# LuizGuzzo/Monocular_Depth_Estimation

Hardware: AMD Instinct MI355X
Metric: training images/sec at 640x480 bs=32/GPU (GuideDepth, SSIM+0.1*L1, Adam) (higher is better)
Workload: dtype fp32; 1 GPU; GuideDepth (DDRNet-23-slim + 3 guided upsampling blocks) train step, BASELINE cfg2, BN in train mode; global_batch=32, per_gpu_batch=32, resolution=640x480, parallelism=dp1

## Files before the change

include/mde_abi.h:

```cpp
#ifndef MDE_ABI_H
#define MDE_ABI_H

#include <stddef.h>
#include <stdint.h>

#ifdef __cplusplus
extern "C" {
#endif

#define MDE_ABI_VERSION 1

#define MDE_F32 0
#define MDE_BF16 1

#define MDE_OK 0
#define MDE_ERR_INVALID_ARG (-1)
#define MDE_ERR_UNSUPPORTED (-2)

int mde_abi_version(void);
const char* mde_status_string(int status);


int mde_bilinear_fwd(const void* x, void* y, int64_t n, int64_t c, int64_t hi,
                     int64_t wi, int64_t ho, int64_t wo, float scale_h,
// ... 64 lines not shown
                        int64_t w, void* workspace, int dtype, void* stream);
int mde_skip_reduce_bn_supported(int64_t cin, int64_t cout, int64_t h, int64_t w, int sums);
size_t mde_skip_reduce_bn_workspace(int64_t n, int64_t cin, int64_t cout, int64_t h, int64_t w);
int mde_skip_reduce_bn_fwd(const void* r, const void* d, const float* in_scale,
                           const float* in_shift, const float* wt, const float* b, void* out,
                           int64_t n, int64_t cin, int64_t cout, int64_t h, int64_t w, int dtype,
                           void* stream);
int mde_skip_reduce_bn_bwd(const void* gout, const void* r, const void* d, const float* in_scale,
                           const float* in_shift, const float* in_mean, const float* wt, void* gs,
                           float* gw, float* gb, float* in_sums, int64_t n, int64_t cin,
                           int64_t cout, int64_t h, int64_t w, void* workspace, int dtype,
                           void* stream);

size_t mde_minmax_workspace(int64_t numel);
int mde_minmax(const void* x, int64_t numel, float* minmax, void* workspace,
               int dtype, void* stream);
int mde_depthnorm_apply(const void* x, const float* minmax, void* y,
                        int64_t numel, int dtype, void* stream);

size_t mde_ssim3_l1_workspace(int64_t b, int64_t h, int64_t w);
int mde_ssim3_l1_fwd(const void* pred, const void* target,
                     const float* target_minmax, float w_ssim, float w_l1,
                     float* loss, void* grad_pred, void* grad_target,
                     int64_t b, int64_t h, int64_t w, void* workspace,
                     int dtype, void* stream);

size_t mde_depth_loss_workspace(int64_t b, int64_t h, int64_t w);
int mde_depth_loss_fwd(const void* pred, const void* gt, float alpha,
                       float beta, float gamma, float max_depth, float* out,
                       int64_t b, int64_t h, int64_t w, void* workspace,
                       int dtype, void* stream);
int mde_depth_loss_bwd(const void* pred, const void* gt, float alpha,
                       float beta, float gamma, float max_depth,
                       const float* fwd_out, const float* gout,
                       void* grad_pred, int64_t b, int64_t h, int64_t w,
                       void* workspace, int dtype, void* stream);

size_t mde_batchnorm_workspace(int64_t n, int64_t c, int64_t h, int64_t w);
int mde_batchnorm_fwd_train(const void* x, const float* gamma, const float* beta,
                            const float* prebias, float* running_mean,
                            float* running_var, int64_t* num_batches_tracked,
                            float momentum, float eps, const void* residual,
                            void* y, float* save_mean, float* save_invstd,
                            int64_t n, int64_t c, int64_t h, int64_t w, int act,
                            void* workspace, int dtype, void* stream);
int mde_batchnorm_fwd_eval(const void* x, const float* gamma, const float* beta,
                           const float* prebias, const float* running_mean,
                           const float* running_var, float eps,
                           const void* residual, void* y, float* save_mean,
                           float* save_invstd, int64_t n, int64_t c, int64_t h,
                           int64_t w, int act, int dtype, void* stream);
int mde_batchnorm_fwd_coef(const void* x, const float* gamma, const float* beta,
                           const float* prebias, float* running_mean, float* running_var,
                           int64_t* num_batches_tracked, float momentum, float eps,
                           int training, float* scale, float* shift, float* save_mean,
                           float* save_invstd, int64_t n, int64_t c, int64_t h, int64_t w,
                           void* workspace, int dtype, void* stream);
int mde_batchnorm_bwd(const void* gy, const void* x, const void* residual,
                      const float* gamma, const float* beta, const float* mean,
                      const float* invstd, int training, void* gx,
                      void* gresidual, float* ggamma, float* gbeta,
                      float* gprebias, int64_t n, int64_t c, int64_t h,
                      int64_t w, int act, void* workspace, int dtype,
                      void* stream);
int mde_batchnorm_fwd_train_stats(const void* x, const float* gamma, const float* beta,
                                  const float* prebias, float* running_mean, float* running_var,
                                  int64_t* num_batches_tracked, float momentum, float eps,
                                  const void* residual, void* y, float* save_mean,
                                  float* save_invstd, int64_t n, int64_t c, int64_t h, int64_t w,
                                  int act, const float* stats, int64_t stats_blocks,
                                  void* workspace, int dtype, void* stream);
int mde_batchnorm_fwd_coef_stats(const void* x, const float* gamma, const float* beta,
                                 const float* prebias, float* running_mean, float* running_var,
                                 int64_t* num_batches_tracked, float momentum, float eps,
                                 float* scale, float* shift, float* save_mean, float* save_invstd,
                                 int64_t n, int64_t c, int64_t h, int64_t w, const float* stats,
                                 int64_t stats_blocks, void* workspace, int dtype, void* stream);
int mde_batchnorm_bwd_apply(const void* gy, const void* x, const void* residual,
                            const float* gamma, const float* beta, const float* mean,
                            const float* invstd, int training, const float* sums, void* gx,
                            void* gresidual, float* ggamma, float* gbeta, float* gprebias,
                            int64_t n, int64_t c, int64_t h, int64_t w, int act, int dtype,
                            void* stream);

size_t mde_window_attn_workspace(int64_t b, int64_t h, int64_t w, int64_t c,
                                 int64_t heads, int64_t window);
int mde_window_attn_fwd(const void* qk, const float* qk_bias, const void* v,
                        const float* v_bias, const float* table, void* out, int64_t b,
                        int64_t h, int64_t w, int64_t c, int64_t heads, int64_t window,
                        int64_t shift, int dtype, void* stream);
int mde_window_attn_bwd(const void* gout, const void* qk, const float* qk_bias,
                        const void* v, const float* v_bias, const float* table, void* gqk,
                        void* gv, float* gtable, float* gqk_bias, float* gv_bias, int64_t b,
                        int64_t h, int64_t w, int64_t c, int64_t heads, int64_t window,
                        int64_t shift, void* workspace, int dtype, void* stream);

size_t mde_colsum_workspace(int64_t t_rows, int64_t n);
int mde_colsum(const void* g, float* gb, int64_t t_rows, int64_t n, void* workspace, int dtype,
               void* stream);
int mde_gelu_bwd_colsum(const void* dh, const void* a, void* da, float* gb, int64_t t_rows,
                        int64_t n, void* workspace, int dtype, void* stream);

size_t mde_linear_wgrad_workspace(int64_t t_rows, int64_t m, int64_t n);
int mde_linear_wgrad(const void* g, const void* x, float* gw, float* gb, int64_t t_rows,
                     int64_t m, int64_t n, void* workspace, int dtype, void* stream);

size_t mde_chansum_workspace(int64_t n, int64_t c, int64_t hw);
int mde_chansum(const void* g, float* gb, int64_t n, int64_t c, int64_t hw, void* workspace,
                int dtype, void* stream);

int mde_head_conv_supported(int64_t n, int64_t c, int64_t h, int64_t w);
int mde_head_conv_fwd(const void* x, const float* weight, const float* bias, void* y, int64_t n,
                      int64_t c, int64_t h, int64_t w, int dtype, void* stream);
int mde_head_conv_dgrad(const void* gy, const float* weight, void* gx, int64_t n, int64_t c,
                        int64_t h, int64_t w, int dtype, void* stream);
size_t mde_head_conv_wgrad_workspace(int64_t n, int64_t c, int64_t h, int64_t w);
int mde_head_conv_wgrad(const void* gy, const void* x, float* gweight, int64_t n, int64_t c,
                        int64_t h, int64_t w, void* workspace, int dtype, void* stream);

int mde_pointwise_supported(int64_t cin, int64_t cout, int64_t h, int64_t w);
size_t mde_pointwise_workspace(int64_t n, int64_t cin, int64_t cout, int64_t h, int64_t w);
int mde_pointwise_fwd(const void* x, const float* in_scale, const float* in_shift,
                      const float* weight, void* y, int64_t n, int64_t cin, int64_t cout,
                      int64_t h, int64_t w, int dtype, void* stream);
int mde_pointwise_bwd(const void* gy, const void* x, const float* in_scale,
                      const float* in_shift, const float* weight, void* gx, float* gweight,
                      int64_t n, int64_t cin, int64_t cout, int64_t h, int64_t w,
                      void* workspace, int dtype, void* stream);
int mde_pointwise_stats_blocks(int64_t n, int64_t cin, int64_t cout, int64_t h, int64_t w);
int mde_pointwise_fwd_stats(const void* x, const float* in_scale, const float* in_shift,
                            const float* weight, void* y, float* stats, int64_t n, int64_t cin,
                            int64_t cout, int64_t h, int64_t w, int dtype, void* stream);
int mde_pointwise_bwd_bn(const void* gy, const void* x, const float* in_scale,
                         const float* in_shift, const float* in_mean, const float* weight,
                         void* gx, float* gweight, float* in_sums, int64_t n, int64_t cin,
                         int64_t cout, int64_t h, int64_t w, void* workspace, int dtype,
                         void* stream);

int mde_conv3x3_supported(int64_t cin, int64_t cout, int pass, int dtype);
int mde_conv3x3_fwd(const void* x, const float* weight, void* y, int64_t n, int64_t cin,
                    int64_t cout, int64_t h, int64_t w, int dtype, void* stream);
int mde_conv3x3_stats_blocks(int64_t n, int64_t cin, int64_t cout, int64_t h, int64_t w,
                             int dtype);
int mde_conv3x3_fwd_stats(const void* x, const float* weight, void* y, float* stats, int64_t n,
                          int64_t cin, int64_t cout, int64_t h, int64_t w, int dtype,
                          void* stream);
int mde_conv3x3_bwd_data(const void* gy, const float* weight, void* gx, int64_t n,
                         int64_t cin, int64_t cout, int64_t h, int64_t w, int dtype,
                         void* stream);
size_t mde_conv3x3_wgrad_workspace(int64_t n, int64_t cin, int64_t cout, int64_t h, int64_t w,
                                   int dtype);
int mde_conv3x3_wgrad(const void* gy, const void* x, float* gweight, int64_t n, int64_t cin,
                      int64_t cout, int64_t h, int64_t w, void* workspace, int dtype,
                      void* stream);

int mde_conv3x3s2_supported(int64_t cin, int64_t cout, int dtype);
size_t mde_conv3x3s2_wgrad_workspace(int64_t n, int64_t cin, int64_t cout, int64_t h, int64_t w,
                                     int dtype);
int mde_conv3x3s2_wgrad(const void* gy, const void* x, float* gweight, int64_t n, int64_t cin,
                        int64_t cout, int64_t h, int64_t w, void* workspace, int dtype,
                        void* stream);

size_t mde_dwconv_workspace(int64_t n, int64_t c, int64_t h, int64_t w, int64_t k,
                            int64_t stride, int64_t pad);
int mde_dwconv_fwd(const void* x, const float* weight, void* y, int64_t n, int64_t c,
                   int64_t h, int64_t w, int64_t k, int64_t stride, int64_t pad, int dtype,
                   void* stream);
int mde_dwconv_bwd(const void* gy, const void* x, const float* weight, void* gx,
                   float* gweight, int64_t n, int64_t c, int64_t h, int64_t w, int64_t k,
                   int64_t stride, int64_t pad, void* workspace, int dtype, void* stream);

size_t mde_layernorm_workspace(int64_t rows, int64_t c);
int mde_layernorm_fwd(const void* x, const float* gamma, const float* beta, void* y,
                      float* mean, float* rstd, int64_t rows, int64_t c, float eps, int dtype,
                      void* stream);
int mde_layernorm_bwd(const void* gy, const void* x, const float* gamma, const float* mean,
                      const float* rstd, void* gx, float* ggamma, float* gbeta, int64_t rows,
                      int64_t c, void* workspace, int dtype, void* stream);
int mde_layernorm_add_fwd(const void* x, const void* r, const float* gamma, const float* beta,
                          void* sum, void* y, float* mean, float* rstd, int64_t rows, int64_t c,
                          float eps, int dtype, void* stream);
int mde_layernorm_bwd_res(const void* gy, const void* x, const void* gres, const float* gamma,
                          const float* mean, const float* rstd, void* gx, float* ggamma,
                          float* gbeta, int64_t rows, int64_t c, void* workspace, int dtype,
                          void* stream);

int mde_transpose(const void* x, void* y, int64_t batch, int64_t m, int64_t n, int dtype,
                  void* stream);

int mde_nyu_augment(const void* image, const void* depth, const int32_t* flags, float* image_out,
                    float* depth_out, int64_t n, int64_t h, int64_t w, int64_t dh, int64_t dw,
                    int depth_bits, void* stream);

size_t mde_eval_workspace(int64_t n, int64_t h, int64_t w);
int mde_eval_sums(const void* pred, const void* gt, int64_t n, int64_t h, int64_t w,
                  float min_depth, float max_depth, int mode, const int32_t* crop,
                  void* workspace, double* sums, int dtype, void* stream);

int mde_conv3x3_guide_bf16_stats_blocks(int64_t n, int64_t cout, int64_t h, int64_t w);
int mde_conv3x3_guide_bf16_fwd(const float* x, const float* weight, void* y, float* stats,
                               int64_t n, int64_t cout, int64_t h, int64_t w, void* stream);

int mde_conv1x1_supported(int64_t cin, int64_t cout, int64_t h, int64_t w, int stride,
                          int dtype);
int mde_conv1x1_fwd(const void* x, const float* weight, void* y, int64_t n, int64_t cin,
                    int64_t cout, int64_t h, int64_t w, int stride, int dtype, void* stream);
int mde_conv1x1_bwd_data(const void* gy, const float* weight, void* gx, int64_t n, int64_t cin,
                         int64_t cout, int64_t h, int64_t w, int stride, int dtype,
                         void* stream);
size_t mde_conv1x1_wgrad_workspace(int64_t n, int64_t cin, int64_t cout, int64_t h, int64_t w,
                                   int stride, int dtype);
int mde_conv1x1_wgrad(const void* gy, const void* x, float* gweight, int64_t n, int64_t cin,
                      int64_t cout, int64_t h, int64_t w, int stride, void* workspace, int dtype,
                      void* stream);

int mde_conv3x3s2_fwd_supported(int64_t cin, int64_t cout, int64_t h, int64_t w, int dtype);
int mde_conv3x3s2_dgrad_supported(int64_t cin, int64_t cout, int64_t h, int64_t w, int dtype);
int mde_conv3x3s2_fwd(const void* x, const float* weight, void* y, int64_t n, int64_t cin,
                      int64_t cout, int64_t h, int64_t w, int dtype, void* stream);
int mde_conv3x3s2_bwd_data(const void* gy, const float* weight, void* gx, int64_t n, int64_t cin,
                           int64_t cout, int64_t h, int64_t w, int dtype, void* stream);

int mde_conv3x3_wide_supported(int64_t cin, int64_t cout, int64_t h, int64_t w, int pass,
                               int dtype);
int mde_conv3x3_wide_fwd(const void* x, const float* weight, void* y, int64_t n, int64_t cin,
                         int64_t cout, int64_t h, int64_t w, int dtype, void* stream);
int mde_conv3x3_wide_bwd_data(const void* gy, const float* weight, void* gx, int64_t n,
                              int64_t cin, int64_t cout, int64_t h, int64_t w, int dtype,
                              void* stream);

int mde_wino_mode(int mode);
int mde_wino_supported(int64_t cin, int64_t cout, int64_t h, int64_t w, int dtype);
size_t mde_wino_weight_bytes(int64_t cin, int64_t cout);
int mde_wino_weight(const float* weight, float* u, int64_t cin, int64_t cout, int flip,
                    void* stream);
int mde_wino_weight2(const float* weight, float* u, float* u_flip, int64_t cin, int64_t cout,
                     void* stream);
// ... 76 lines not shown
```

monocular_depth_estimation_amd/_abi.py:

```python
from __future__ import annotations

import ctypes
import os

import torch

LIB_PATH = os.environ.get("MDE_HIP_LIB") or os.path.join(
    os.path.dirname(os.path.abspath(__file__)), "libmde_hip.so")

MDE_F32 = 0
MDE_BF16 = 1

_c = ctypes
_vp = _c.c_void_p
_i64 = _c.c_int64
_f32 = _c.c_float
_int = _c.c_int
_sz = _c.c_size_t
_fp = _c.POINTER(_c.c_float)

SIGNATURES = {
    "mde_abi_version": (_int, []),
    "mde_status_string": (_c.c_char_p, [_int]),
    "mde_bilinear_fwd": (_int, [_vp, _vp, _i64, _i64, _i64, _i64, _i64, _i64, _f32, _f32, _int, _int, _vp]),
    "mde_bilinear_bwd": (_int, [_vp, _vp, _i64, _i64, _i64, _i64, _i64, _i64, _f32, _f32, _int, _int, _vp]),
    "mde_bilinear_bwd2_supported": (_int, [_i64, _i64, _i64, _i64, _i64, _i64, _f32, _f32, _int]),
    "mde_bilinear_bwd2": (_int, [_vp, _vp, _vp, _i64, _i64, _i64, _i64, _i64, _i64, _f32, _f32, _int,
                                 _int, _vp]),
    "mde_nearest_fwd": (_int, [_vp, _vp, _i64, _i64, _i64, _i64, _i64, _i64, _f32, _f32, _int, _vp]),
    "mde_nearest_bwd": (_int, [_vp, _vp, _i64, _i64, _i64, _i64, _i64, _i64, _f32, _f32, _int, _vp]),
    "mde_nearest_pyramid_supported": (_int, [_i64, _i64, _i64, _i64]),
    "mde_nearest_pyramid": (_int, [_vp, _vp, _vp, _i64, _i64, _i64, _i64, _int, _vp]),
    "mde_se_workspace": (_sz, [_i64, _i64, _i64, _i64, _i64]),
    "mde_se_fwd": (_int, [_vp, _i64, _vp, _i64, _vp, _vp, _i64, _vp, _vp, _vp, _vp,
                          _i64, _i64, _i64, _vp, _int, _vp]),
    "mde_se_bwd": (_int, [_vp, _vp, _i64, _vp, _i64, _vp, _vp, _i64, _vp, _vp, _vp,
                          _vp, _vp, _vp, _vp, _i64, _i64, _i64, _vp, _int, _vp]),
    "mde_se_bn_workspace": (_sz, [_i64, _i64, _i64, _i64, _i64]),
    "mde_se_bn_fwd": (_int, [_vp, _i64, _vp, _i64, _vp, _vp, _vp, _vp, _i64, _vp, _vp, _vp, _vp,
                             _i64, _i64, _i64, _vp, _int, _vp]),
    "mde_se_bn_bwd": (_int, [_vp, _vp, _i64, _vp, _i64, _vp, _vp, _vp, _vp, _int, _vp, _vp, _i64,
                             _vp, _vp, _vp, _vp, _vp, _vp, _vp, _vp, _vp, _i64, _i64, _i64, _vp,
                             _int, _vp]),
    "mde_skip_reduce_fwd": (_int, [_vp, _vp, _vp, _vp, _vp, _i64, _i64, _i64, _i64, _i64, _int, _vp]),
    "mde_skip_reduce_workspace": (_sz, [_i64, _i64, _i64, _i64, _i64]),
    "mde_skip_reduce_bwd": (_int, [_vp, _vp, _vp, _vp, _vp, _vp, _vp, _i64, _i64, _i64, _i64, _i64,
                                   _vp, _int, _vp]),
    "mde_skip_reduce_bn_supported": (_int, [_i64, _i64, _i64, _i64, _int]),
    "mde_skip_reduce_bn_workspace": (_sz, [_i64, _i64, _i64, _i64, _i64]),
    "mde_skip_reduce_bn_fwd": (_int, [_vp, _vp, _vp, _vp, _vp, _vp, _vp, _i64, _i64, _i64, _i64, _i64,
                                      _int, _vp]),
    "mde_skip_reduce_bn_bwd": (_int, [_vp, _vp, _vp, _vp, _vp, _vp, _vp, _vp, _vp, _vp, _vp, _i64,
                                      _i64, _i64, _i64, _i64, _vp, _int, _vp]),
    "mde_minmax_workspace": (_sz, [_i64]),
    "mde_minmax": (_int, [_vp, _i64, _vp, _vp, _int, _vp]),
    "mde_depthnorm_apply": (_int, [_vp, _vp, _vp, _i64, _int, _vp]),
    "mde_ssim3_l1_workspace": (_sz, [_i64, _i64, _i64]),
    "mde_ssim3_l1_fwd": (_int, [_vp, _vp, _vp, _f32, _f32, _vp, _vp, _vp, _i64, _i64, _i64, _vp, _int, _vp]),
    "mde_depth_loss_workspace": (_sz, [_i64, _i64, _i64]),
    "mde_depth_loss_fwd": (_int, [_vp, _vp, _f32, _f32, _f32, _f32, _vp, _i64, _i64, _i64, _vp, _int, _vp]),
    "mde_depth_loss_bwd": (_int, [_vp, _vp, _f32, _f32, _f32, _f32, _vp, _vp, _vp, _i64, _i64, _i64,
                                  _vp, _int, _vp]),
    "mde_batchnorm_workspace": (_sz, [_i64, _i64, _i64, _i64]),
    "mde_batchnorm_fwd_train": (_int, [_vp, _vp, _vp, _vp, _vp, _vp, _vp, _f32, _f32, _vp, _vp, _vp,
                                       _vp, _i64, _i64, _i64, _i64, _int, _vp, _int, _vp]),
    "mde_batchnorm_fwd_eval": (_int, [_vp, _vp, _vp, _vp, _vp, _vp, _f32, _vp, _vp, _vp, _vp,
                                      _i64, _i64, _i64, _i64, _int, _int, _vp]),
    "mde_batchnorm_bwd": (_int, [_vp, _vp, _vp, _vp, _vp, _vp, _vp, _int, _vp, _vp, _vp, _vp, _vp,
                                 _i64, _i64, _i64, _i64, _int, _vp, _int, _vp]),
    "mde_batchnorm_bwd_apply": (_int, [_vp, _vp, _vp, _vp, _vp, _vp, _vp, _int, _vp, _vp, _vp, _vp,
                                       _vp, _vp, _i64, _i64, _i64, _i64, _int, _int, _vp]),
    "mde_window_attn_workspace": (_sz, [_i64, _i64, _i64, _i64, _i64, _i64]),
    "mde_window_attn_fwd": (_int, [_vp, _vp, _vp, _vp, _vp, _vp, _i64, _i64, _i64, _i64, _i64, _i64,
                                   _i64, _int, _vp]),
    "mde_window_attn_bwd": (_int, [_vp, _vp, _vp, _vp, _vp, _vp, _vp, _vp, _vp, _vp, _vp, _i64, _i64,
                                   _i64, _i64, _i64, _i64, _i64, _vp, _int, _vp]),
    "mde_se_gate_fwd": (_int, [_vp, _i64, _vp, _i64, _vp, _vp, _vp, _vp, _i64, _int, _vp, _vp, _vp,
                               _vp, _i64, _i64, _i64, _vp, _int, _vp]),
    "mde_se_gate_bwd": (_int, [_vp, _vp, _i64, _vp, _i64, _vp, _vp, _vp, _i64, _int, _vp, _vp, _vp,
                               _vp, _vp, _vp, _vp, _vp, _vp, _i64, _i64, _i64, _vp, _int, _vp]),
    "mde_pointwise_supported": (_int, [_i64, _i64, _i64, _i64]),
    "mde_pointwise_workspace": (_sz, [_i64, _i64, _i64, _i64, _i64]),
    "mde_pointwise_fwd": (_int, [_vp, _vp, _vp, _vp, _vp, _i64, _i64, _i64, _i64, _i64, _int, _vp]),
    "mde_pointwise_bwd": (_int, [_vp, _vp, _vp, _vp, _vp, _vp, _vp, _i64, _i64, _i64, _i64, _i64,
                                 _vp, _int, _vp]),
    "mde_pointwise_stats_blocks": (_int, [_i64, _i64, _i64, _i64, _i64]),
    "mde_pointwise_fwd_stats": (_int, [_vp, _vp, _vp, _vp, _vp, _vp, _i64, _i64, _i64, _i64, _i64,
                                       _int, _vp]),
    "mde_conv3x3_stats_blocks": (_int, [_i64, _i64, _i64, _i64, _i64, _int]),
    "mde_conv3x3_fwd_stats": (_int, [_vp, _vp, _vp, _vp, _i64, _i64, _i64, _i64, _i64, _int, _vp]),
    "mde_batchnorm_fwd_train_stats": (_int, [_vp, _vp, _vp, _vp, _vp, _vp, _vp, _f32, _f32, _vp,
                                             _vp, _vp, _vp, _i64, _i64, _i64, _i64, _int, _vp,
                                             _i64, _vp, _int, _vp]),
    "mde_batchnorm_fwd_coef_stats": (_int, [_vp, _vp, _vp, _vp, _vp, _vp, _vp, _f32, _f32, _vp,
                                            _vp, _vp, _vp, _i64, _i64, _i64, _i64, _vp, _i64, _vp,
                                            _int, _vp]),
    "mde_pointwise_bwd_bn": (_int, [_vp, _vp, _vp, _vp, _vp, _vp, _vp, _vp, _vp, _i64, _i64, _i64,
                                    _i64, _i64, _vp, _int, _vp]),
    "mde_batchnorm_fwd_coef": (_int, [_vp, _vp, _vp, _vp, _vp, _vp, _vp, _f32, _f32, _int, _vp, _vp,
                                      _vp, _vp, _i64, _i64, _i64, _i64, _vp, _int, _vp]),
    "mde_conv3x3_supported": (_int, [_i64, _i64, _int, _int]),
    "mde_conv3x3_fwd": (_int, [_vp, _vp, _vp, _i64, _i64, _i64, _i64, _i64, _int, _vp]),
    "mde_conv3x3_bwd_data": (_int, [_vp, _vp, _vp, _i64, _i64, _i64, _i64, _i64, _int, _vp]),
    "mde_conv3x3_wgrad_workspace": (_sz, [_i64, _i64, _i64, _i64, _i64, _int]),
    "mde_conv3x3_wgrad": (_int, [_vp, _vp, _vp, _i64, _i64, _i64, _i64, _i64, _vp, _int, _vp]),
    "mde_conv3x3s2_supported": (_int, [_i64, _i64, _int]),
    "mde_conv3x3s2_wgrad_workspace": (_sz, [_i64, _i64, _i64, _i64, _i64, _int]),
    "mde_conv3x3s2_wgrad": (_int, [_vp, _vp, _vp, _i64, _i64, _i64, _i64, _i64, _vp, _int, _vp]),
    "mde_dwconv_workspace": (_sz, [_i64, _i64, _i64, _i64, _i64, _i64, _i64]),
    "mde_dwconv_fwd": (_int, [_vp, _vp, _vp, _i64, _i64, _i64, _i64, _i64, _i64, _i64, _int, _vp]),
    "mde_dwconv_bwd": (_int, [_vp, _vp, _vp, _vp, _vp, _i64, _i64, _i64, _i64, _i64, _i64, _i64,
                              _vp, _int, _vp]),
    "mde_layernorm_workspace": (_sz, [_i64, _i64]),
    "mde_layernorm_fwd": (_int, [_vp, _vp, _vp, _vp, _vp, _vp, _i64, _i64, _f32, _int, _vp]),
    "mde_layernorm_bwd": (_int, [_vp, _vp, _vp, _vp, _vp, _vp, _vp, _vp, _i64, _i64, _vp, _int,
                                 _vp]),
    "mde_layernorm_add_fwd": (_int, [_vp, _vp, _vp, _vp, _vp, _vp, _vp, _vp, _i64, _i64, _f32,
                                      _int, _vp]),
    "mde_layernorm_bwd_res": (_int, [_vp, _vp, _vp, _vp, _vp, _vp, _vp, _vp, _vp, _i64, _i64,
                                      _vp, _int, _vp]),
    "mde_transpose": (_int, [_vp, _vp, _i64, _i64, _i64, _int, _vp]),
    "mde_nyu_augment": (_int, [_vp, _vp, _vp, _vp, _vp, _i64, _i64, _i64, _i64, _i64, _int, _vp]),
    "mde_eval_workspace": (_sz, [_i64, _i64, _i64]),
    "mde_eval_sums": (_int, [_vp, _vp, _i64, _i64, _i64, _f32, _f32, _int, _c.POINTER(_c.c_int32), _vp,
                             _vp, _int, _vp]),
    "mde_colsum_workspace": (_sz, [_i64, _i64]),
    "mde_colsum": (_int, [_vp, _vp, _i64, _i64, _vp, _int, _vp]),
    "mde_head_conv_supported": (_int, [_i64, _i64, _i64, _i64]),
    "mde_head_conv_fwd": (_int, [_vp, _vp, _vp, _vp, _i64, _i64, _i64, _i64, _int, _vp]),
    "mde_head_conv_dgrad": (_int, [_vp, _vp, _vp, _i64, _i64, _i64, _i64, _int, _vp]),
    "mde_head_conv_wgrad_workspace": (_sz, [_i64, _i64, _i64, _i64]),
    "mde_head_conv_wgrad": (_int, [_vp, _vp, _vp, _i64, _i64, _i64, _i64, _vp, _int, _vp]),
    "mde_chansum_workspace": (_sz, [_i64, _i64, _i64]),
    "mde_chansum": (_int, [_vp, _vp, _i64, _i64, _i64, _vp, _int, _vp]),
    "mde_linear_wgrad_workspace": (_sz, [_i64, _i64, _i64]),
    "mde_linear_wgrad": (_int, [_vp, _vp, _vp, _vp, _i64, _i64, _i64, _vp, _int, _vp]),
    "mde_gelu_bwd_colsum": (_int, [_vp, _vp, _vp, _vp, _i64, _i64, _vp, _int, _vp]),
    "mde_conv1x1_supported": (_int, [_i64, _i64, _i64, _i64, _int, _int]),
    "mde_conv1x1_fwd": (_int, [_vp, _vp, _vp, _i64, _i64, _i64, _i64, _i64, _int, _int, _vp]),
    "mde_conv1x1_bwd_data": (_int, [_vp, _vp, _vp, _i64, _i64, _i64, _i64, _i64, _int, _int, _vp]),
    "mde_conv1x1_wgrad_workspace": (_sz, [_i64, _i64, _i64, _i64, _i64, _int, _int]),
    "mde_conv1x1_wgrad": (_int, [_vp, _vp, _vp, _i64, _i64, _i64, _i64, _i64, _int, _vp, _int,
                                 _vp]),
    "mde_conv3x3s2_fwd_supported": (_int, [_i64, _i64, _i64, _i64, _int]),
    "mde_conv3x3s2_dgrad_supported": (_int, [_i64, _i64, _i64, _i64, _int]),
    "mde_conv3x3s2_fwd": (_int, [_vp, _vp, _vp, _i64, _i64, _i64, _i64, _i64, _int, _vp]),
    "mde_conv3x3s2_bwd_data": (_int, [_vp, _vp, _vp, _i64, _i64, _i64, _i64, _i64, _int, _vp]),
    "mde_conv3x3_wide_supported": (_int, [_i64, _i64, _i64, _i64, _int, _int]),
    "mde_conv3x3_wide_fwd": (_int, [_vp, _vp, _vp, _i64, _i64, _i64, _i64, _i64, _int, _vp]),
    "mde_conv3x3_wide_bwd_data": (_int, [_vp, _vp, _vp, _i64, _i64, _i64, _i64, _i64, _int, _vp]),
    "mde_wino_mode": (_int, [_int]),
    "mde_wino_supported": (_int, [_i64, _i64, _i64, _i64, _int]),
    "mde_wino_weight_bytes": (_sz, [_i64, _i64]),
    "mde_wino_weight": (_int, [_vp, _vp, _i64, _i64, _int, _vp]),
    "mde_wino_weight2": (_int, [_vp, _vp, _vp, _i64, _i64, _vp]),
    "mde_wino_weight_blocks": (_i64, [_i64, _i64, _int]),
    "mde_wino_weight_table": (_int, [_vp, _int, _i64, _i64, _vp]),
    "mde_wino_conv": (_int, [_vp, _vp, _vp, _i64, _i64, _i64, _i64, _i64, _int, _int, _vp]),
    "mde_wino_conv_acc": (_int, [_vp, _vp, _vp, _vp, _i64, _i64, _i64, _i64, _i64, _int, _int, _vp]),
    "mde_wino_conv_stats": (_int, [_vp, _vp, _vp, _vp, _i64, _i64, _i64, _i64, _i64, _int, _int,
                                   _vp]),
    "mde_wino_stats_blocks": (_int, [_i64, _i64, _i64, _i64, _i64]),
    "mde_batchnorm_stats_route": (_int, [_i64, _i64, _i64, _i64, _i64, _int]),
    "mde_bn_chan_mode": (_int, [_int]),
    "mde_convbf_supported": (_int, [_i64, _i64, _i64, _i64, _int, _int, _int]),
    "mde_convbf_supported_n": (_int, [_i64, _i64, _i64, _i64, _i64, _int, _int, _int]),
    "mde_convbf_flops": (_c.c_double, [_i64, _i64, _i64, _i64, _i64, _int, _int, _int]),
    "mde_stem_bf16_supported": (_int, [_i64, _i64, _i64, _i64]),
    "mde_stem_bf16_fwd": (_int, [_vp, _vp, _vp, _i64, _i64, _i64, _i64, _vp]),
    "mde_stem_bf16_wgrad_workspace": (_sz, [_i64, _i64, _i64, _i64]),
    "mde_stem_bf16_wgrad": (_int, [_vp, _vp, _vp, _i64, _i64, _i64, _i64, _vp, _vp]),
    "mde_conv3x3_guide_bf16_wgrad_workspace": (_sz, [_i64, _i64, _i64, _i64]),
    "mde_conv3x3_guide_bf16_wgrad": (_int, [_vp, _vp, _vp, _i64, _i64, _i64, _i64, _vp, _vp]),
    "mde_convbf_pack_elems": (_sz, [_i64, _i64, _int, _int]),
    "mde_convbf_pack": (_int, [_vp, _vp, _i64, _i64, _int, _int, _vp]),
    "mde_convbf_pack_both": (_int, [_vp, _vp, _vp, _i64, _i64, _int, _vp]),
    "mde_convbf_pack_table": (_int, [_vp, _int, _i64, _i64, _vp]),
    "mde_convbf_stats_blocks": (_int, [_i64, _i64, _i64, _i64, _i64, _int, _int]),
    "mde_convbf_fwd": (_int, [_vp, _vp, _vp, _vp, _i64, _i64, _i64, _i64, _i64, _int, _int, _vp]),
    "mde_convbf_bwd_data": (_int, [_vp, _vp, _vp, _i64, _i64, _i64, _i64, _i64, _int, _int, _vp]),
    "mde_convbf_wgrad_workspace": (_sz, [_i64, _i64, _i64, _i64, _i64, _int, _int]),
    "mde_convbf_wgrad": (_int, [_vp, _vp, _vp, _i64, _i64, _i64, _i64, _i64, _int, _int, _vp, _vp]),
    "mde_conv3x3_guide_bf16_stats_blocks": (_int, [_i64, _i64, _i64, _i64]),
    "mde_conv3x3_guide_bf16_fwd": (_int, [_vp, _vp, _vp, _vp, _i64, _i64, _i64, _i64, _vp]),
    "mde_graph_count_memsets": (_int, [_vp, _c.POINTER(_i64)]),
    "mde_graph_replace_memsets": (_int, [_vp, _c.POINTER(_i64)]),
    "mde_graph_node_counts": (_int, [_vp, _c.POINTER(_i64)]),
    "mde_graph_node_types": (_int, [_vp, _c.POINTER(_i64)]),
# ... 153 lines not shown
```

monocular_depth_estimation_amd/csrc/bn.hip:

```cpp
#include <cmath>

#include <cstdlib>
#include <type_traits>

#include "common.h"

namespace {

constexpr int kTarget = 2048;
constexpr int kMinSlice = 4096;
constexpr int kPlaneChunk4 = 1024;
constexpr int64_t kMaxApplyRecords = 256;

struct Geo {
  int64_t c, hw, total;
  int slices;
  int64_t slice_len;
};

int64_t env_or(const char* name, int64_t dflt) {
  const char* v = std::getenv(name);
  return v && *v ? std::atoll(v) : dflt;
}

// ... 411 lines not shown
};

struct BwdCh {
  float sc, sh, A, B, D;
};

__device__ BwdCh bwd_channel(const BwdArgs& P, int64_t ch, double sdy,
                             double sdyx, bool owner) {
  BwdCh r;
  const double is = (double)P.invstd[ch];
  const double mu = (double)P.mean[ch];
  const double scale = (double)P.gamma[ch] * is;
  double A = scale, B = 0.0, D = 0.0;
  const double n = (double)P.total;
  if (P.training) {
    B = -scale * is * is * sdyx / n;
    D = -scale * sdy / n - B * mu;
  }
  if (owner) {
    if (P.ggamma) P.ggamma[ch] = (float)(sdyx * is);
    if (P.gbeta) P.gbeta[ch] = (float)sdy;
    if (P.gprebias) P.gprebias[ch] = (float)(A * sdy + B * n * mu + D * n);
  }
  r.sc = P.gamma[ch] * P.invstd[ch];
  r.sh = P.beta[ch] - P.mean[ch] * r.sc;
  r.A = (float)A;
  r.B = (float)B;
  r.D = (float)D;
  return r;
}

template <typename T>
__global__ void __launch_bounds__(256)
    bn_bwd_apply_plane_kernel(const T* __restrict__ gy, const T* __restrict__ x,
                              const T* __restrict__ r, T* __restrict__ gx,
                              T* __restrict__ gr, int64_t c, int64_t hw, int act,
                              BwdArgs P) {
  __shared__ float cf[5];
  const int64_t plane = blockIdx.y;
  const int64_t ch = plane % c;
  const int64_t hw4 = hw >> 2;
  const T* gp = gy + plane * hw;
  const T* xp = x + plane * hw;
  const T* rp = r ? r + plane * hw : nullptr;
  T* op = gx + plane * hw;
  T* orp = gr ? gr + plane * hw : nullptr;
  const int64_t b0 = blockIdx.x * (int64_t)kPlaneChunk4;
  constexpr int KK = kPlaneChunk4 / 256;
  float4 g4[KK], v4[KK], q4[KK];
#pragma unroll
  for (int k = 0; k < KK; ++k) {
    const int64_t i = b0 + k * 256 + threadIdx.x;
    const int64_t ic = i < hw4 ? i : hw4 - 1;
    g4[k] = ld4_nt(gp + 4 * ic);
    v4[k] = ld4_nt(xp + 4 * ic);
    q4[k] = rp ? ld4_nt(rp + 4 * ic) : make_float4(0.f, 0.f, 0.f, 0.f);
  }
  if (threadIdx.x < 64) {
    double a, b;
    wave_slices(P.part, ch, P.slices, &a, &b);
    if (threadIdx.x == 0) {
      const BwdCh k = bwd_channel(P, ch, a, b, blockIdx.x == 0 && plane < c);
      cf[0] = k.sc; cf[1] = k.sh; cf[2] = k.A; cf[3] = k.B; cf[4] = k.D;
    }
  }
  __syncthreads();
  const float sc = cf[0], sh = cf[1], A = cf[2], B = cf[3], D = cf[4];
#pragma unroll
  for (int k = 0; k < KK; ++k) {
    const int64_t i = b0 + k * 256 + threadIdx.x;
    if (i < hw4) {
      const float4 g = g4[k], v = v4[k], q = q4[k];
      const float4 e = make_float4(dy_eff(g.x, v.x, q.x, sc, sh, act),
                                   dy_eff(g.y, v.y, q.y, sc, sh, act),
                                   dy_eff(g.z, v.z, q.z, sc, sh, act),
                                   dy_eff(g.w, v.w, q.w, sc, sh, act));
      st4_nt(op + 4 * i, make_float4(A * e.x + B * v.x + D, A * e.y + B * v.y + D,
                                     A * e.z + B * v.z + D, A * e.w + B * v.w + D));
      if (orp) st4_nt(orp + 4 * i, e);
    }
  }
}

template <typename T>
__global__ void __launch_bounds__(256)
    bn_bwd_apply_table_kernel(const T* __restrict__ gy, const T* __restrict__ x,
                              const T* __restrict__ r, T* __restrict__ gx,
                              T* __restrict__ gr, int64_t planes, int64_t c,
                              int64_t hw, int act, BwdArgs P) {
  extern __shared__ float tab[];
  const PlaneShare ps(planes, c);
  for (int64_t kk = threadIdx.x; kk < ps.nch; kk += blockDim.x) {
    const int64_t ch = ps.channel(kk, c);
    double a = 0.0, b = 0.0;
    for (int s = 0; s < P.slices; ++s) {
      a += (double)P.part[(ch * P.slices + s) * 2];
      b += (double)P.part[(ch * P.slices + s) * 2 + 1];
    }
    const BwdCh k = bwd_channel(P, ch, a, b, ps.owner(ch));
    tab[ch] = k.sc;
    tab[c + ch] = k.sh;
    tab[2 * c + ch] = k.A;
    tab[3 * c + ch] = k.B;
    tab[4 * c + ch] = k.D;
  }
  __syncthreads();
  const int64_t total = planes * hw;
  if (table_vec(total, hw)) {
    const uint32_t hw4 = (uint32_t)(hw >> 2), cc = (uint32_t)c;
    const uint32_t t1 = (uint32_t)(ps.p1 * (hw >> 2));
    for (uint32_t t = (uint32_t)(ps.p0 * (hw >> 2)) + threadIdx.x; t < t1; t += blockDim.x) {
      const uint32_t ch = (t / hw4) % cc;
      const int64_t o = 4 * (int64_t)t;
      const float sc = tab[ch], sh = tab[c + ch];
      const float A = tab[2 * c + ch], B = tab[3 * c + ch], D = tab[4 * c + ch];
      const float4 v = ld4(x + o), g = ld4(gy + o);
      const float4 q = r ? ld4(r + o) : make_float4(0.f, 0.f, 0.f, 0.f);
      float4 e, o4;
      e.x = dy_eff(g.x, v.x, q.x, sc, sh, act);
      e.y = dy_eff(g.y, v.y, q.y, sc, sh, act);
      e.z = dy_eff(g.z, v.z, q.z, sc, sh, act);
      e.w = dy_eff(g.w, v.w, q.w, sc, sh, act);
      o4.x = A * e.x + B * v.x + D;
      o4.y = A * e.y + B * v.y + D;
      o4.z = A * e.z + B * v.z + D;
      o4.w = A * e.w + B * v.w + D;
      st4(gx + o, o4);
      if (gr) st4(gr + o, e);
    }
    return;
  }
  for (int64_t t = ps.p0 * hw + threadIdx.x; t < ps.p1 * hw; t += blockDim.x) {
    const int64_t ch = (t / hw) % c;
    const float v = ld1(x + t);
    const float e = dy_eff(ld1(gy + t), v, r ? ld1(r + t) : 0.f, tab[ch], tab[c + ch], act);
    st1(gx + t, tab[2 * c + ch] * e + tab[3 * c + ch] * v + tab[4 * c + ch]);
    if (gr) st1(gr + t, e);
  }
}

constexpr int kChanThreads = 512;
constexpr int kChanUnits = 8;
constexpr int64_t kChanMax = (int64_t)kChanThreads * kChanUnits * 4;

int g_chan_mode = [] {
  const char* e = std::getenv("MDE_BN_CHAN");
  return e ? std::atoi(e) : 2;
}();

template <typename T>
inline bool chan_mode(int64_t n, int64_t hw) {
  const bool on = std::is_same_v<T, float> ? g_chan_mode >= 1 : g_chan_mode >= 2;
  return on && !plane_mode(hw) && n * hw <= (hw % 4 == 0 ? kChanMax : kChanMax / 4);
}

__device__ __forceinline__ void chan_sum2(double* a, double* b, double (*red)[kChanThreads / 64]) {
  const int lane = threadIdx.x & 63, wv = threadIdx.x >> 6;
  double x = wave_sum_d(*a), y = wave_sum_d(*b);
  if (lane == 0) {
    red[0][wv] = x;
    red[1][wv] = y;
  }
  __syncthreads();
  x = 0.0;
  y = 0.0;
#pragma unroll
// ... 460 lines not shown
  if (!dtype_ok(dtype)) return MDE_ERR_UNSUPPORTED;
  if (!x || !gamma || !beta || !y || !save_mean || !save_invstd || !workspace || !stats ||
      stats_blocks <= 0 || stats_blocks > 0x7fffffff || (!running_mean != !running_var) ||
      act < 0 || act > 2 || !args_ok(n, c, h, w))
    return MDE_ERR_INVALID_ARG;
  hipStream_t s = (hipStream_t)stream;
  const int64_t hw = h * w;
  if (dtype == MDE_BF16 ? chan_mode<bf16>(n, hw) : chan_mode<float>(n, hw))
    return mde_batchnorm_fwd_train(x, gamma, beta, prebias, running_mean, running_var,
                                   num_batches_tracked, momentum, eps, residual, y, save_mean,
                                   save_invstd, n, c, h, w, act, workspace, dtype, stream);
  float* part = (float*)workspace;
  if (plane_mode(hw) && stats_blocks <= kMaxApplyRecords) {
    FwdArgs A{gamma, beta, prebias, part, 0, n * hw, hw, eps, momentum, running_mean,
              running_var, num_batches_tracked, save_mean, save_invstd, 1, stats,
              (int)stats_blocks};
    if (dtype == MDE_BF16)
      return launch_fwd_apply((const bf16*)x, (const bf16*)residual, (bf16*)y, n, c, hw, act, A, s);
    return launch_fwd_apply((const float*)x, (const float*)residual, (float*)y, n, c, hw, act, A, s);
  }
  const double mb = 16.0 * (double)c * stats_blocks;
  if (dtype == MDE_BF16)
    MDE_LAUNCH(mde::K_BN_FINAL, mb, s, (bn_stats_merge_kernel<bf16, false>), dim3((unsigned)c),
               dim3(256), 0, (const bf16*)x, stats, (int)stats_blocks, hw, part, FwdArgs{},
               nullptr, nullptr);
  else
    MDE_LAUNCH(mde::K_BN_FINAL, mb, s, (bn_stats_merge_kernel<float, false>), dim3((unsigned)c),
               dim3(256), 0, (const float*)x, stats, (int)stats_blocks, hw, part, FwdArgs{},
               nullptr, nullptr);
  FwdArgs A{gamma, beta, prebias, part, 1, n * hw, hw, eps, momentum,
            running_mean, running_var, num_batches_tracked, save_mean, save_invstd, 1};
  if (dtype == MDE_BF16)
    return launch_fwd_apply((const bf16*)x, (const bf16*)residual, (bf16*)y, n, c, hw, act, A, s);
  return launch_fwd_apply((const float*)x, (const float*)residual, (float*)y, n, c, hw, act, A, s);
}

int mde_batchnorm_fwd_coef_stats(const void* x, const float* gamma, const float* beta,
                                 const float* prebias, float* running_mean, float* running_var,
                                 int64_t* num_batches_tracked, float momentum, float eps,
                                 float* scale, float* shift, float* save_mean, float* save_invstd,
                                 int64_t n, int64_t c, int64_t h, int64_t w, const float* stats,
                                 int64_t stats_blocks, void* workspace, int dtype, void* stream) {
  if (!dtype_ok(dtype)) return MDE_ERR_UNSUPPORTED;
  if (!x || !gamma || !beta || !scale || !shift || !save_mean || !save_invstd || !workspace ||
      !stats || stats_blocks <= 0 || stats_blocks > 0x7fffffff ||
      (!running_mean != !running_var) || !args_ok(n, c, h, w))
    return MDE_ERR_INVALID_ARG;
  hipStream_t s = (hipStream_t)stream;
  const int64_t hw = h * w;
  float* part = (float*)workspace;
  const double mb = 16.0 * (double)c * stats_blocks;
  FwdArgs A{gamma, beta, prebias, part, 1, n * hw, hw, eps, momentum, running_mean, running_var,
            num_batches_tracked, save_mean, save_invstd, 1};
  if (dtype == MDE_BF16) {
    MDE_LAUNCH(mde::K_BN_FINAL, mb + 8.0 * (double)c, s, (bn_stats_merge_kernel<bf16, true>),
               dim3((unsigned)c), dim3(256), 0, (const bf16*)x, stats, (int)stats_blocks, hw,
               part, A, scale, shift);
  } else {
    MDE_LAUNCH(mde::K_BN_FINAL, mb + 8.0 * (double)c, s, (bn_stats_merge_kernel<float, true>),
               dim3((unsigned)c), dim3(256), 0, (const float*)x, stats, (int)stats_blocks, hw,
               part, A, scale, shift);
  }
  return MDE_OK;
}

int mde_batchnorm_bwd_apply(const void* gy, const void* x, const void* residual,
                            const float* gamma, const float* beta, const float* mean,
                            const float* invstd, int training, const float* sums, void* gx,
                            void* gresidual, float* ggamma, float* gbeta, float* gprebias,
                            int64_t n, int64_t c, int64_t h, int64_t w, int act, int dtype,
                            void* stream) {
  if (!dtype_ok(dtype)) return MDE_ERR_UNSUPPORTED;
  if (!gy || !x || !gamma || !beta || !mean || !invstd || !sums || !gx || act < 0 || act > 2 ||
      !args_ok(n, c, h, w) || (gresidual && !residual && act))
    return MDE_ERR_INVALID_ARG;
  hipStream_t s = (hipStream_t)stream;
  const int64_t hw = h * w;
  BwdArgs P{gamma, beta, mean, invstd, sums, 1, n * hw, training, ggamma, gbeta, gprebias};
  return dtype == MDE_BF16
             ? bwd_apply<bf16>(gy, x, residual, gx, gresidual, n, c, hw, act, P, s)
             : bwd_apply<float>(gy, x, residual, gx, gresidual, n, c, hw, act, P, s);
}

}
```

monocular_depth_estimation_amd/csrc/conv3x3.hip:

```cpp
#include <cstdlib>

#include "common.h"

namespace {

using f4 = __attribute__((__vector_size__(4 * sizeof(float)))) float;

__device__ __forceinline__ f4 mfma4(float a, float b, f4 c) {
  return __builtin_amdgcn_mfma_f32_16x16x4f32(a, b, c, 0, 0, 0);
}

__device__ __forceinline__ int clampi(int v, int lo, int hi) { return v < lo ? lo : (v > hi ? hi : v); }

template <auto Kernel>
int resident_blocks() {
  static const int cached = [] {
    int dev = 0, cus = 0, per = 0;
    (void)hipGetDevice(&dev);
    (void)hipDeviceGetAttribute(&cus, hipDeviceAttributeMultiprocessorCount, dev);
    (void)hipOccupancyMaxActiveBlocksPerMultiprocessor(&per, Kernel, 256, 0);
    return (cus > 0 ? cus : 256) * (per > 0 ? per : 1);
  }();
  return cached;
}

constexpr int kTW = 64;
constexpr int kXW = kTW + 2;

constexpr int cpad4(int c) { return (c + 3) / 4 * 4; }
constexpr int plane_words(int rows, int mod) { return (rows * kXW + 63) / 64 * 64 + mod; }
constexpr int wrow_words(int co) { return co == 16 ? 16 : (co == 32 ? 48 : 80); }

__device__ __forceinline__ float rbf(float v) {
  return __uint_as_float((uint32_t)__builtin_bit_cast(uint16_t, (__bf16)v) << 16);
}

template <int CI, int CIP, int XR>
struct HaloTile {
  static constexpr int ROWS = CIP * XR;
  static constexpr int RPWV = (ROWS + 3) / 4;
  static constexpr int NH = (2 * RPWV + 63) / 64;
  static_assert(RPWV <= 64 && NH <= 32, "mask widths");
  float a[RPWV];
  float b[NH];
  uint64_t am;
  unsigned bm;

  __device__ __forceinline__ void load(const float* __restrict__ xi, int h, int w, int r0,
                                       int c0, int lane, int wvu) {
    const int gc = c0 - 1 + lane;
    const bool cok = gc >= 0 && gc < w;
    am = 0;
#pragma unroll
    for (int k = 0; k < RPWV; ++k) {
      const int ri = wvu + 4 * k;
      const int c = ri / XR, r = ri % XR, gr = r0 - 1 + r;
      const bool ok = (ROWS % 4 == 0 || ri < ROWS) && (CI == CIP || c < CI) && gr >= 0 &&
                      gr < h && cok;
      a[k] = xi[ok ? (unsigned)((c * h + gr) * w + gc) : 0u];
      am |= ok ? (uint64_t)1 << k : (uint64_t)0;
    }
    bm = 0;
#pragma unroll
    for (int q = 0; q < NH; ++q) {
      const int e = 64 * q + lane;
      const int ri = wvu + 4 * (e >> 1);
      const int c = ri / XR, r = ri % XR, gr = r0 - 1 + r, g2 = c0 + 63 + (e & 1);
      const bool ok = e < 2 * RPWV && ri < ROWS && c < CI && gr >= 0 && gr < h && g2 < w;
      b[q] = xi[ok ? (unsigned)((c * h + gr) * w + g2) : 0u];
      bm |= ok ? 1u << q : 0u;
    }
  }

  template <int PS, bool RB = false>
  __device__ __forceinline__ void store(float* sx, int lane, int wvu) const {
#pragma unroll
    for (int k = 0; k < RPWV; ++k) {
      const int ri = wvu + 4 * k;
      if (ROWS % 4 == 0 || ri < ROWS) {
        const float v = (am >> k) & 1 ? a[k] : 0.f;
        sx[(ri / XR) * PS + (ri % XR) * kXW + lane] = RB ? rbf(v) : v;
      }
    }
#pragma unroll
    for (int q = 0; q < NH; ++q) {
      const int e = 64 * q + lane;
      const int ri = wvu + 4 * (e >> 1);
      if (e < 2 * RPWV && ri < ROWS) {
        const float v = (bm >> q) & 1u ? b[q] : 0.f;
        sx[(ri / XR) * PS + (ri % XR) * kXW + 64 + (e & 1)] = RB ? rbf(v) : v;
      }
    }
  }
};

template <int CO, int TH, bool FULL>
struct GradTile {
  static constexpr int ROWS = CO * TH;
  static constexpr int PER = (ROWS + 15) / 16;
  static_assert(PER <= 32, "mask width");
  float4 v[PER];
  unsigned vm;

  __device__ __forceinline__ void load(const float* __restrict__ gi, int h, int w, int r0,
                                       int c0, int lane, int wvu) {
    const int gc = c0 + 4 * (lane & 15);
    vm = 0;
#pragma unroll
    for (int i = 0; i < PER; ++i) {
      const int ri = 16 * i + 4 * wvu + (lane >> 4);
      const int c = ri / TH, gr = r0 + ri % TH;
      const bool rok = (ROWS % 16 == 0 || ri < ROWS) && gr < h;
      if constexpr (FULL) {
        v[i] = *reinterpret_cast<const float4*>(gi + (rok ? (unsigned)((c * h + gr) * w + gc) : 0u));
        vm |= rok ? 1u << i : 0u;
      } else {
        const float* src = gi + (rok ? ((int64_t)c * h + gr) * w + gc : 0);
        const bool vec = (w & 3) == 0 && gc + 3 < w;
        if (vec) {
          const float4 t = *reinterpret_cast<const float4*>(src);
          v[i] = rok ? t : make_float4(0.f, 0.f, 0.f, 0.f);
        } else {
          float4 t;
          t.x = rok && gc < w ? src[0] : 0.f;
          t.y = rok && gc + 1 < w ? src[1] : 0.f;
          t.z = rok && gc + 2 < w ? src[2] : 0.f;
          t.w = rok && gc + 3 < w ? src[3] : 0.f;
          v[i] = t;
        }
      }
    }
  }

  template <int PSG>
  __device__ __forceinline__ void store(float* sg, int lane, int wvu) const {
#pragma unroll
    for (int i = 0; i < PER; ++i) {
      const int ri = 16 * i + 4 * wvu + (lane >> 4);
      if (ROWS % 16 == 0 || ri < ROWS) {
        float4 t = v[i];
        if (FULL && !((vm >> i) & 1u)) t = make_float4(0.f, 0.f, 0.f, 0.f);
        *reinterpret_cast<float4*>(sg + (ri / TH) * PSG + (ri % TH) * kTW + 4 * (lane & 15)) = t;
      }
    }
  }
};

struct TileGeo {
  int img, r0, c0;
};

struct TileWalk {
  int t0, step, end;
};

__device__ __forceinline__ TileWalk tile_walk(int ntiles) {
  const int b = blockIdx.x, g = gridDim.x;
  if (g % 8 != 0 || ntiles < g) return {b, g, ntiles};
  const int span = (ntiles + 7) / 8, grp = b & 7;
  const int end = (grp + 1) * span < ntiles ? (grp + 1) * span : ntiles;
  return {grp * span + (b >> 3), g >> 3, end};
}

__device__ __forceinline__ TileGeo tile_geo(int tile, int th, int tiles_w, int tiles_per_img) {
  const int t = tile % tiles_per_img;
  return {tile / tiles_per_img, (t / tiles_w) * th, (t % tiles_w) * kTW};
}

template <int CI, int CO, int RPW, bool FLIP, bool STATS = false, typename TO = float>
__global__ void __launch_bounds__(256, 2)
    conv3x3_fwd_kernel(const float* __restrict__ x, const float* __restrict__ wt,
                       TO* __restrict__ y, int h, int w, int tiles_w, int tiles_per_img,
                       int ntiles, float* __restrict__ stats = nullptr) {
  static_assert(!(STATS && FLIP), "statistics are a forward epilogue");
  constexpr bool RB = sizeof(TO) == 2;
  constexpr int CIP = cpad4(CI);
  constexpr int TH = 4 * RPW;
  constexpr int XR = TH + 2;
  constexpr int PS = plane_words(XR, 16);
  constexpr int WS = wrow_words(CO);
  constexpr int NB = CO / 16;
  __shared__ float sx[CIP * PS];
  __shared__ float sw[9 * CIP * WS];
  constexpr int kSOL = 64 + 16 / (int)sizeof(TO);
  constexpr bool SO = CI == 3 && !FLIP && TH * CO * kSOL * (int)sizeof(TO) <= 40 * 1024;
  __shared__ __attribute__((aligned(16))) TO so[SO ? TH * CO * kSOL : 4];

  const int tid = threadIdx.x, lane = tid & 63, wv = tid >> 6;
  const int wvu = __builtin_amdgcn_readfirstlane(wv);
  const int64_t img_in = (int64_t)CI * h * w, img_out = (int64_t)CO * h * w;

  {
    constexpr int WN = 9 * CIP * CO;
    constexpr int WPER = (WN + 255) / 256;
    float v[WPER];
#pragma unroll
    for (int i = 0; i < WPER; ++i) {
      const int e = tid + 256 * i;
      const int co = e % CO, rest = e / CO, ci = rest % CIP, tap = rest / CIP;
      const bool ok = e < WN && ci < CI;
      const int src = FLIP ? (ci * CO + co) * 9 + (8 - tap) : (co * CI + ci) * 9 + tap;
      const float t = wt[ok ? src : 0];
      v[i] = ok ? (RB ? rbf(t) : t) : 0.f;
    }
#pragma unroll
    for (int i = 0; i < WPER; ++i) {
      const int e = tid + 256 * i;
      const int co = e % CO, rest = e / CO, ci = rest % CIP, tap = rest / CIP;
      if (e < WN) sw[(tap * CIP + ci) * WS + co] = v[i];
    }
  }

  const int li = lane & 15, lk = lane >> 4;
  const float* ax = sx + lk * PS + li + wv * RPW * kXW;
  const float* bw = sw + lk * WS + li;
  const bool vec = (w & 3) == 0;

  mde::Sh run[STATS ? NB : 1];
#pragma unroll
  for (int nb = 0; nb < (STATS ? NB : 1); ++nb) run[nb] = {0.f, 0.f, 0.f, 0.f};
  bool first = true;
  HaloTile<CI, CIP, XR> T;
  const TileWalk tw = tile_walk(ntiles);
  int tile = tw.t0;
  if (tile < tw.end) {
    const TileGeo g = tile_geo(tile, TH, tiles_w, tiles_per_img);
    T.load(x + g.img * img_in, h, w, g.r0, g.c0, lane, wvu);
  }
  for (; tile < tw.end; tile += tw.step) {
    const TileGeo g = tile_geo(tile, TH, tiles_w, tiles_per_img);
    __syncthreads();
    T.template store<PS, RB>(sx, lane, wvu);
    __syncthreads();
    const int nxt = tile + tw.step;
    if (nxt < tw.end) {
      const TileGeo gn = tile_geo(nxt, TH, tiles_w, tiles_per_img);
      T.load(x + gn.img * img_in, h, w, gn.r0, gn.c0, lane, wvu);
    }

    f4 acc[RPW][4][NB];
#pragma unroll
    for (int q = 0; q < RPW; ++q)
#pragma unroll
      for (int m = 0; m < 4; ++m)
#pragma unroll
        for (int nb = 0; nb < NB; ++nb) acc[q][m][nb] = f4{0.f, 0.f, 0.f, 0.f};
#pragma unroll
    for (int tap = 0; tap < 9; ++tap) {
      const int dy = tap / 3, dx = tap % 3;
#pragma unroll
      for (int cs = 0; cs < CIP / 4; ++cs) {
        float b[NB];
#pragma unroll
        for (int nb = 0; nb < NB; ++nb) b[nb] = bw[(tap * CIP + 4 * cs) * WS + nb * 16];
#pragma unroll
        for (int q = 0; q < RPW; ++q)
#pragma unroll
          for (int m = 0; m < 4; ++m) {
            const float a = ax[4 * cs * PS + (q + dy) * kXW + m * 16 + dx];
#pragma unroll
            for (int nb = 0; nb < NB; ++nb) acc[q][m][nb] = mfma4(a, b[nb], acc[q][m][nb]);
          }
      }
    }

    if constexpr (RB) {
#pragma unroll
      for (int q = 0; q < RPW; ++q)
#pragma unroll
        for (int m = 0; m < 4; ++m)
#pragma unroll
          for (int nb = 0; nb < NB; ++nb)
#pragma unroll
            for (int i = 0; i < 4; i += 2) {
              using bf2v = __bf16 __attribute__((ext_vector_type(2)));
              const uint32_t p = __builtin_bit_cast(
                  uint32_t, bf2v{(__bf16)acc[q][m][nb][i], (__bf16)acc[q][m][nb][i + 1]});
              acc[q][m][nb][i] = __uint_as_float(p << 16);
              acc[q][m][nb][i + 1] = __uint_as_float(p & 0xffff0000u);
            }
    }
    if constexpr (STATS) {
#pragma unroll
      for (int nb = 0; nb < NB; ++nb) {
        if (first) {
          const bool ok0 = g.r0 + wv * RPW < h && g.c0 < w;
          run[nb].ref = __shfl(ok0 ? acc[0][0][nb][0] : 0.f, li, 64);
        }
#pragma unroll
        for (int q = 0; q < RPW; ++q) {
          const int row = g.r0 + wv * RPW + q;
          if (row < h && g.c0 + 64 <= w) {
#pragma unroll
            for (int m = 0; m < 4; ++m)
#pragma unroll
              for (int i = 0; i < 4; ++i) {
                const float d = acc[q][m][nb][i] - run[nb].ref;
                run[nb].s1 += d;
                run[nb].s2 = fmaf(d, d, run[nb].s2);
              }
            run[nb].n += 16.f;
          } else {
#pragma unroll
            for (int m = 0; m < 4; ++m)
#pragma unroll
              for (int i = 0; i < 4; ++i) {
                const int col = g.c0 + m * 16 + 4 * lk + i;
                mde::sh_add(run[nb], acc[q][m][nb][i], row < h && col < w);
              }
          }
        }
      }
      first = false;
    }
    TO* yi = y + g.img * img_out;
    if constexpr (SO) {
      if (vec) {
#pragma unroll
        for (int q = 0; q < RPW; ++q)
#pragma unroll
          for (int m = 0; m < 4; ++m)
// ... 22 lines not shown
          const uint4 u = *reinterpret_cast<const uint4*>(so + line * kSOL + PX * pc);
          TO* dst = yi + ((int64_t)co * h + grow) * w + col;
          if (grow < h && col + PX <= w)
            *reinterpret_cast<uint4*>(dst) = u;
          else if (grow < h && col < w)
            *reinterpret_cast<uint2*>(dst) = make_uint2(u.x, u.y);
        }
        continue;
      }
    }
#pragma unroll
    for (int q = 0; q < RPW; ++q) {
      const int row = g.r0 + wv * RPW + q;
      if (row >= h) continue;
#pragma unroll
      for (int m = 0; m < 4; ++m) {
        const int col = g.c0 + m * 16 + 4 * lk;
#pragma unroll
        for (int nb = 0; nb < NB; ++nb) {
          TO* dst = yi + ((int64_t)(nb * 16 + li) * h + row) * w + col;
          const f4 v = acc[q][m][nb];
          if (vec && col + 3 < w) {
            mde::st4(dst, make_float4(v[0], v[1], v[2], v[3]));
          } else {
#pragma unroll
            for (int i = 0; i < 4; ++i)
              if (col + i < w) mde::st1(dst + i, v[i]);
          }
        }
      }
    }
  }
  if constexpr (STATS) {
    __syncthreads();
    float* part = sx;
#pragma unroll
    for (int nb = 0; nb < NB; ++nb) {
      const mde::Sh a = mde::sh_xor_sum(mde::sh_xor_sum(run[nb], 16), 32);
      if (lk == 0) {
        float* p4 = part + (wv * CO + 16 * nb + li) * 4;
        p4[0] = a.ref;
        p4[1] = a.n;
        p4[2] = a.s1;
        p4[3] = a.s2;
      }
    }
    __syncthreads();
    if (tid < CO) {
      mde::Sh a{part[tid * 4], part[tid * 4 + 1], part[tid * 4 + 2], part[tid * 4 + 3]};
#pragma unroll
      for (int k = 1; k < 4; ++k) {
        const float* p4 = part + (k * CO + tid) * 4;
        a = mde::sh_merge(a, {p4[0], p4[1], p4[2], p4[3]});
      }
      float* o4 = stats + ((int64_t)tid * gridDim.x + blockIdx.x) * 4;
      o4[0] = a.ref;
      o4[1] = a.n;
      o4[2] = a.s1;
      o4[3] = a.s2;
    }
  }
}

template <int CI, int CO, int TH, int PW>
struct WgradCfg {
  static constexpr int CIP = cpad4(CI);
  static constexpr int XR = TH + 2;
  static constexpr int PSX = plane_words(XR, 4);
  static constexpr int PSG = TH * kTW + 4;
  static constexpr int NREAL = 9 * CIP;
  static constexpr int NP = (NREAL + 15) / 16 * 16;
  static constexpr int NBLK = NP / 16;
  static constexpr int MB = CO / 16;
  static constexpr int TWAYS = 4 / PW;
  static constexpr int NBW = (NBLK + TWAYS - 1) / TWAYS;
  static constexpr int RPWG = TH / PW;
  static constexpr int ZERO = CIP * PSX;
  static constexpr int STAGE = ZERO + XR * kXW + CO * PSG;
  static constexpr int RED = PW == 1 ? 0 : PW * MB * NBLK * 256;
  static constexpr int SMEM = STAGE > RED ? STAGE : RED;
  static constexpr int M = CO * NP;
};

template <int CI, int CO, int TH, int PW, bool FULL>
__global__ void __launch_bounds__(256, 2)
    conv3x3_wgrad_kernel(const float* __restrict__ x, const float* __restrict__ gy,
                         float* __restrict__ part, int h, int w, int tiles_w,
                         int tiles_per_img, int ntiles) {
  using C = WgradCfg<CI, CO, TH, PW>;
  __shared__ float smem[C::SMEM];
  float* sx = smem;
  float* sg = smem + C::ZERO + C::XR * kXW;

  const int tid = threadIdx.x, lane = tid & 63, wv = tid >> 6;
  const int li = lane & 15, lk = lane >> 4;
  const int pg = wv % PW, tg = wv / PW;
  const int wvu = __builtin_amdgcn_readfirstlane(wv);
  const int64_t img_in = (int64_t)CI * h * w, img_out = (int64_t)CO * h * w;

  int boff[C::NBW];
#pragma unroll
  for (int j = 0; j < C::NBW; ++j) {
    const int n = 16 * (tg + C::TWAYS * j) + li;
    if (n < C::NREAL) {
      const int tap = n / C::CIP, ci = n % C::CIP;
      boff[j] = ci * C::PSX + (tap / 3) * kXW + tap % 3 + lk;
    } else {
      boff[j] = C::ZERO + lk;
    }
  }
  const int aoff = li * C::PSG + lk;

  f4 acc[C::MB][C::NBW];
#pragma unroll
  for (int mb = 0; mb < C::MB; ++mb)
#pragma unroll
    for (int j = 0; j < C::NBW; ++j) acc[mb][j] = f4{0.f, 0.f, 0.f, 0.f};

  for (int e = tid; e < C::XR * kXW; e += 256) smem[C::ZERO + e] = 0.f;
  HaloTile<CI, C::CIP, C::XR> T;
  GradTile<CO, TH, FULL> G;
  const TileWalk tw = tile_walk(ntiles);
  int tile = tw.t0;
  if (tile < tw.end) {
    const TileGeo g = tile_geo(tile, TH, tiles_w, tiles_per_img);
    G.load(gy + g.img * img_out, h, w, g.r0, g.c0, lane, wvu);
    T.load(x + g.img * img_in, h, w, g.r0, g.c0, lane, wvu);
  }
  for (; tile < tw.end; tile += tw.step) {
    __syncthreads();
    T.template store<C::PSX>(sx, lane, wvu);
    G.template store<C::PSG>(sg, lane, wvu);
    __syncthreads();
    const int nxt = tile + tw.step;
    if (nxt < tw.end) {
      const TileGeo gn = tile_geo(nxt, TH, tiles_w, tiles_per_img);
      G.load(gy + gn.img * img_out, h, w, gn.r0, gn.c0, lane, wvu);
      T.load(x + gn.img * img_in, h, w, gn.r0, gn.c0, lane, wvu);
    }

    for (int rr = 0; rr < C::RPWG; ++rr) {
      const int row = pg * C::RPWG + rr;
      const float* ga = sg + aoff + row * kTW;
      const float* xb = sx + row * kXW;
#pragma unroll 4
      for (int s = 0; s < kTW / 4; ++s) {
        float a[C::MB];
#pragma unroll
        for (int mb = 0; mb < C::MB; ++mb) a[mb] = ga[mb * 16 * C::PSG + 4 * s];
#pragma unroll
        for (int j = 0; j < C::NBW; ++j) {
          const float b = xb[boff[j] + 4 * s];
#pragma unroll
          for (int mb = 0; mb < C::MB; ++mb) acc[mb][j] = mfma4(a[mb], b, acc[mb][j]);
        }
      }
    }
  }

  float* out = part + (int64_t)blockIdx.x * C::M;
  if constexpr (PW == 1) {
#pragma unroll
    for (int mb = 0; mb < C::MB; ++mb)
#pragma unroll
      for (int j = 0; j < C::NBW; ++j) {
        const int nb = tg + C::TWAYS * j;
        if (nb < C::NBLK) {
#pragma unroll
          for (int i = 0; i < 4; ++i)
            out[(16 * mb + 4 * lk + i) * C::NP + 16 * nb + li] = acc[mb][j][i];
        }
      }
    return;
  }
  __syncthreads();
#pragma unroll
  for (int mb = 0; mb < C::MB; ++mb)
#pragma unroll
    for (int j = 0; j < C::NBW; ++j) {
      const int nb = tg + C::TWAYS * j;
      if (nb < C::NBLK) {
        float* d = smem + ((pg * C::MB + mb) * C::NBLK + nb) * 256 + li;
#pragma unroll
        for (int i = 0; i < 4; ++i) d[(4 * lk + i) * 16] = acc[mb][j][i];
      }
    }
  __syncthreads();
  for (int e = tid; e < C::M; e += 256) {
    const int co = e / C::NP, n = e % C::NP;
    const int mb = co / 16, nb = n / 16;
    const int o = ((mb * C::NBLK + nb) * 256) + (co % 16) * 16 + n % 16;
    float s = 0.f;
#pragma unroll
    for (int p = 0; p < PW; ++p) s += smem[p * C::MB * C::NBLK * 256 + o];
    out[e] = s;
  }
}

struct ReduceMap {
  int wide;
  int np, cip;
  int ci_n, co_n;
};

__device__ __forceinline__ int64_t gw_index(const ReduceMap& r, int grp, int e) {
  if (r.wide) {
    const int ngo = r.co_n / r.wide, col = e / 288, n = e % 288;
    const int co = (grp % ngo) * r.wide + col, ci = (grp / ngo) * 32 + n % 32;
    if (ci >= r.ci_n) return -1;
    return ((int64_t)co * r.ci_n + ci) * 9 + n / 32;
  }
  const int co = e / r.np, n = e % r.np, tap = n / r.cip, ci = n % r.cip;
  if (tap >= 9 || ci >= r.ci_n) return -1;
  return ((int64_t)co * r.ci_n + ci) * 9 + tap;
}

constexpr int kRedWaves = 16;

__global__ void __launch_bounds__(64 * kRedWaves)
    wgrad_reduce_kernel(const float* __restrict__ part, float* __restrict__ gw, int g, int m,
                        ReduceMap map) {
  __shared__ float red[kRedWaves][64];
// ... 1347 lines not shown
    if (lane < C::XRW) {
      const int rk = wvu + 4 * lane;
      if (rk < C::XR) sx[(rk / 3) * C::PSX + (rk % 3) * C::RW] = hok ? xh : 0.f;
    }
    G.template store<C::PSG>(sg, lane, wvu);
    __syncthreads();
    const int nxt = tile + tw.step;
    if (nxt < tw.end) load(nxt);
#pragma unroll
    for (int st = 0; st < 16 / C::KW; ++st) {
      const int s4 = 4 * (kw + C::KW * st);
      float a[C::MTW];
#pragma unroll
      for (int i = 0; i < C::MTW; ++i) a[i] = sg[aoff[i] + s4];
#pragma unroll
      for (int j = 0; j < C::NTW; ++j) {
        const float b = sx[boff[j] + s4];
#pragma unroll
        for (int i = 0; i < C::MTW; ++i) acc[i][j] = mfma4(a[i], b, acc[i][j]);
      }
    }
  }
  float* out = part + (int64_t)blockIdx.x * C::M;
  if constexpr (C::KW == 1) {
#pragma unroll
    for (int i = 0; i < C::MTW; ++i)
#pragma unroll
      for (int j = 0; j < C::NTW; ++j) {
        const int mt = mw * C::MTW + i, nt = nw * C::NTW + j;
#pragma unroll
        for (int q = 0; q < 4; ++q) out[(16 * mt + 4 * lk + q) * C::NP + 16 * nt + li] = acc[i][j][q];
      }
    return;
  }
  __syncthreads();
#pragma unroll
  for (int i = 0; i < C::MTW; ++i)
#pragma unroll
    for (int j = 0; j < C::NTW; ++j) {
      const int mt = mw * C::MTW + i, nt = nw * C::NTW + j;
      float* d = smem + ((kw * C::MT + mt) * C::NT + nt) * 256 + li;
#pragma unroll
      for (int q = 0; q < 4; ++q) d[(4 * lk + q) * 16] = acc[i][j][q];
    }
  __syncthreads();
  for (int e = tid; e < C::M; e += 256) {
    const int co = e / C::NP, n = e % C::NP;
    const int o = ((co / 16) * C::NT + n / 16) * 256 + (co % 16) * 16 + n % 16;
    float sum = 0.f;
#pragma unroll
    for (int k = 0; k < C::KW; ++k) sum += smem[k * C::MT * C::NT * 256 + o];
    out[e] = sum;
  }
}

enum Pass { kFwd = 0, kDgrad = 1, kWgrad = 2 };

template <int CI, int CO, int RPW, bool FLIP, bool STATS = false, typename TO = float>
int fwd_grid(int64_t n, int64_t h, int64_t w, int* tiles_w, int* tiles_per_img, int* ntiles) {
  constexpr int TH = 4 * RPW;
  *tiles_w = (int)mde::cdiv(w, kTW);
  *tiles_per_img = (int)(mde::cdiv(h, TH) * *tiles_w);
  const int64_t nt = n * *tiles_per_img;
  if (nt > 0x7fffffff) return 0;
  *ntiles = (int)nt;
  const int res = resident_blocks<conv3x3_fwd_kernel<CI, CO, RPW, FLIP, STATS, TO>>();
  return nt < res ? (int)nt : res;
}

template <int CI, int CO, int RPW, bool FLIP, bool STATS = false, typename TO = float>
int launch_fwd(const float* in, const float* wt, TO* out, int64_t n, int64_t h, int64_t w,
               double bytes, int kid, hipStream_t s, float* stats = nullptr) {
  const double flops = 2.0 * 9 * CI * CO * (double)(n * h * w);
  int tiles_w, tiles_per_img, ntiles;
  const int grid =
      fwd_grid<CI, CO, RPW, FLIP, STATS, TO>(n, h, w, &tiles_w, &tiles_per_img, &ntiles);
  if (grid <= 0) return MDE_ERR_INVALID_ARG;
  MDE_LAUNCH_MFMA(kid, bytes, flops, s, (conv3x3_fwd_kernel<CI, CO, RPW, FLIP, STATS, TO>),
                  dim3(grid), dim3(256), 0, in, wt, out, (int)h, (int)w, tiles_w, tiles_per_img,
                  ntiles, stats);
  return MDE_OK;
}

struct WgradPlan {
  int th, tiles_w, tiles_per_img, ntiles, grid, m, np, cip;
};

constexpr int kWgradGrid = 1024;

template <int CI, int CO, int TH, int PW>
WgradPlan wgrad_plan(int64_t n, int64_t h, int64_t w) {
  using C = WgradCfg<CI, CO, TH, PW>;
  WgradPlan p;
  p.th = TH;
  p.tiles_w = (int)mde::cdiv(w, kTW);
  p.tiles_per_img = (int)(mde::cdiv(h, TH) * p.tiles_w);
  const int64_t nt = n * p.tiles_per_img;
  p.ntiles = nt > 0x7fffffff ? 0x7fffffff : (int)nt;
  p.grid = p.ntiles < kWgradGrid ? p.ntiles : kWgradGrid;
  p.m = C::M;
  p.np = C::NP;
  p.cip = C::CIP;
  return p;
}

template <int CI, int CO, int TH, int PW>
int launch_wgrad(const float* x, const float* gy, float* gw, int64_t n, int64_t h, int64_t w,
                 float* ws, double bytes, hipStream_t s) {
  const WgradPlan p = wgrad_plan<CI, CO, TH, PW>(n, h, w);
  const double flops = 2.0 * 9 * CI * CO * (double)(n * h * w);
  if (CI == 3) {
    if (w % kTW == 0)
      MDE_LAUNCH(mde::K_C3_WGRAD_GUIDE, bytes, s, (conv3x3_wgrad_kernel<CI, CO, TH, PW, true>),
                 dim3(p.grid), dim3(256), 0, x, gy, ws, (int)h, (int)w, p.tiles_w,
                 p.tiles_per_img, p.ntiles);
    else
      MDE_LAUNCH(mde::K_C3_WGRAD_GUIDE, bytes, s, (conv3x3_wgrad_kernel<CI, CO, TH, PW, false>),
                 dim3(p.grid), dim3(256), 0, x, gy, ws, (int)h, (int)w, p.tiles_w,
                 p.tiles_per_img, p.ntiles);
  } else if (w % kTW == 0) {
    MDE_LAUNCH_MFMA(mde::K_C3_WGRAD, bytes, flops, s, (conv3x3_wgrad_kernel<CI, CO, TH, PW, true>),
                    dim3(p.grid), dim3(256), 0, x, gy, ws, (int)h, (int)w, p.tiles_w,
                    p.tiles_per_img, p.ntiles);
  } else {
    MDE_LAUNCH_MFMA(mde::K_C3_WGRAD, bytes, flops, s, (conv3x3_wgrad_kernel<CI, CO, TH, PW, false>),
                    dim3(p.grid), dim3(256), 0, x, gy, ws, (int)h, (int)w, p.tiles_w,
                    p.tiles_per_img, p.ntiles);
  }
  return launch_reduce(ws, gw, 1, p.grid, p.m, ReduceMap{0, p.np, p.cip, CI, CO}, s);
}

struct S2Plan {
  int ho, wo, tiles_w, tiles_per_img, ntiles, grid, m, np, cip;
};

template <int CI, int CO>
S2Plan s2_plan(int64_t n, int64_t h, int64_t w) {
  using C = S2Cfg<CI, CO>;
  S2Plan p;
  p.ho = (int)((h - 1) / 2 + 1);
  p.wo = (int)((w - 1) / 2 + 1);
  p.tiles_w = (int)mde::cdiv(p.wo, kTW);
  p.tiles_per_img = p.ho * p.tiles_w;
  const int64_t nt = n * p.tiles_per_img;
  p.ntiles = nt > 0x7fffffff ? 0x7fffffff : (int)nt;
  const int res = resident_blocks<conv3x3s2_wgrad_kernel<CI, CO, false>>();
  p.grid = p.ntiles < res ? p.ntiles : res;
  p.m = C::M;
  p.np = C::NP;
  p.cip = C::CIP;
  return p;
}

bool s2_supported(int64_t cin, int64_t cout) {
  return (cin == 3 || cin == 32) && cout == 32;
}

template <int CI, int CO>
int launch_wgrad_s2(const float* x, const float* gy, float* gw, int64_t n, int64_t h, int64_t w,
                    float* ws, hipStream_t s) {
  const S2Plan p = s2_plan<CI, CO>(n, h, w);
  if (p.grid <= 0) return MDE_ERR_INVALID_ARG;
  const double flops = 2.0 * 9 * CI * CO * (double)n * p.ho * p.wo;
  const double bytes = 4.0 * (double)n * ((double)CI * h * w + (double)CO * p.ho * p.wo);
  if (p.wo % kTW == 0)
    MDE_LAUNCH_MFMA(mde::K_C3_WGRAD_S2, bytes, flops, s, (conv3x3s2_wgrad_kernel<CI, CO, true>),
                    dim3(p.grid), dim3(256), 0, x, gy, ws, (int)h, (int)w, p.ho, p.wo, p.tiles_w,
                    p.tiles_per_img, p.ntiles);
  else
    MDE_LAUNCH_MFMA(mde::K_C3_WGRAD_S2, bytes, flops, s, (conv3x3s2_wgrad_kernel<CI, CO, false>),
                    dim3(p.grid), dim3(256), 0, x, gy, ws, (int)h, (int)w, p.ho, p.wo, p.tiles_w,
                    p.tiles_per_img, p.ntiles);
  return launch_reduce(ws, gw, 1, p.grid, p.m, ReduceMap{0, p.np, p.cip, CI, CO}, s);
}

inline bool bf_v2(int64_t h, int64_t w) {
  static const bool on = [] {
    const char* e = std::getenv("MDE_C3BF_V2");
    return !(e && e[0] == '0');
  }();
  return on && w % 4 == 0 && 2 * 32 * h * w < (int64_t)1 << 30;
}

template <int CI, int CO, int RPW, bool FLIP, bool STATS>
int bf_fwd_grid(int64_t n, int64_t h, int64_t w, int* tiles_w, int* tiles_per_img, int* ntiles) {
  constexpr int TH = 4 * RPW;
  *tiles_w = (int)mde::cdiv(w, kTW);
  *tiles_per_img = (int)(mde::cdiv(h, TH) * *tiles_w);
  const int64_t nt = n * *tiles_per_img;
  if (nt > 0x7fffffff) return 0;
  *ntiles = (int)nt;
  const int res = bf_v2(h, w) ? resident_blocks<conv3x3_bf_fwd2_kernel<CI, CO, RPW, FLIP, STATS>>()
                           : resident_blocks<conv3x3_bf_fwd_kernel<CI, CO, RPW, FLIP, STATS>>();
  return nt < res ? (int)nt : res;
}

inline int bf_rpw_forced() {
  static const int r = [] {
    const char* e = std::getenv("MDE_BF_RPW");
    return e && (e[0] == '1' || e[0] == '2') ? e[0] - '0' : 0;
  }();
  return r;
}
inline int bf_rpw(int64_t ch) {
  const int f = bf_rpw_forced();
  return f ? f : (ch == 16 ? 2 : 1);
}

template <int CI, int CO, int RPW, bool FLIP, bool STATS = false>
int launch_bf_fwd(const bf16* in, const float* wt, bf16* out, int64_t n, int64_t h, int64_t w,
                  double bytes, int kid, hipStream_t s, float* stats = nullptr) {
  const double flops = 2.0 * 9 * CI * CO * (double)(n * h * w);
  int tiles_w, tiles_per_img, ntiles;
  const int grid =
// ... 219 lines not shown
                                 mde::K_C3_DGRAD_BF16, s)
    if (cin == 16) return bf_rpw(16) == 2 ? MDE_BF(16, 2) : MDE_BF(16, 1);
    return bf_rpw(32) == 2 ? MDE_BF(32, 2) : MDE_BF(32, 1);
#undef MDE_BF
  }
  if (dtype != MDE_F32) return MDE_ERR_UNSUPPORTED;
  if (!gy || !weight || !gx || !dims_ok(n, h, w)) return MDE_ERR_INVALID_ARG;
  if (!supported(cin, cout, kDgrad)) return MDE_ERR_UNSUPPORTED;
  hipStream_t s = (hipStream_t)stream;
  const float* in = (const float*)gy;
  float* out = (float*)gx;
  const double bytes = 4.0 * n * h * w * (double)(cin + cout);
  const int k = mde::K_C3_DGRAD;
  if (cin == 16 && variant() == 1) return launch_fwd<16, 16, 2, true>(in, weight, out, n, h, w, bytes, k, s);
  if (cin == 16) return launch_fwd<16, 16, 1, true>(in, weight, out, n, h, w, bytes, k, s);
  return launch_fwd<32, 32, 1, true>(in, weight, out, n, h, w, bytes, k, s);
}

size_t mde_conv3x3_wgrad_workspace(int64_t n, int64_t cin, int64_t cout, int64_t h, int64_t w,
                                   int dtype) {
  WgradPlan p;
  if (dtype == MDE_BF16) {
    if (!bf_supported(cin, cout) || !dims_ok(n, h, w)) return 0;
    p = cin == 16 ? bf_wgrad_plan<16, 16, 4, 4>(n, h, w) : bf_wgrad_plan<32, 32, 2, 2>(n, h, w);
    return wgrad_ws_bytes(1, p.grid, p.m);
  }
  if (!supported(cin, cout, kWgrad) || !dims_ok(n, h, w)) return 0;
  if (wide(cin, cout) || wide_pad(cin, cout)) {
    WidePlan wp;
    return wide_plan(n, cin, cout, h, w, &wp) ? wide_workspace(wp) : 0;
  }
  if (cin == 3 && cout == 16) p = wgrad_plan<3, 16, 8, 4>(n, h, w);
  else if (cin == 3 && cout == 32) p = wgrad_plan<3, 32, 8, 4>(n, h, w);
  else if (cin == 3) p = wgrad_plan<3, 64, 4, 4>(n, h, w);
  else if (cin == 16 && variant() == 1) p = wgrad_plan<16, 16, 8, 4>(n, h, w);
  else if (cin == 16 && variant() == 2) p = wgrad_plan<16, 16, 4, 2>(n, h, w);
  else if (cin == 16) p = wgrad_plan<16, 16, 4, 4>(n, h, w);
  else if (c32_wide(w)) {
    const WidePlan wp = c32_plan(n, h, w);
    return wgrad_ws_bytes(1, wp.gx, WideT<1, 80, 1, 32>::M);
  } else if (variant() == 1) p = wgrad_plan<32, 32, 4, 2>(n, h, w);
  else if (variant() == 2) p = wgrad_plan<32, 32, 4, 1>(n, h, w);
  else p = wgrad_plan<32, 32, 2, 2>(n, h, w);
  return wgrad_ws_bytes(1, p.grid, p.m);
}

int mde_conv3x3_wgrad(const void* gy, const void* x, float* gweight, int64_t n, int64_t cin,
                      int64_t cout, int64_t h, int64_t w, void* workspace, int dtype,
                      void* stream) {
  if (dtype == MDE_BF16) {
    if (!gy || !x || !gweight || !workspace || !dims_ok(n, h, w) || w % 4)
      return MDE_ERR_INVALID_ARG;
    if (!bf_supported(cin, cout)) return MDE_ERR_UNSUPPORTED;
    hipStream_t s = (hipStream_t)stream;
    const double bytes = 2.0 * n * h * w * (double)(cin + cout);
    if (cin == 16)
      return launch_bf_wgrad<16, 16, 4, 4>((const bf16*)x, (const bf16*)gy, gweight, n, h, w,
                                           (float*)workspace, bytes, s);
    return launch_bf_wgrad<32, 32, 2, 2>((const bf16*)x, (const bf16*)gy, gweight, n, h, w,
                                         (float*)workspace, bytes, s);
  }
  if (dtype != MDE_F32) return MDE_ERR_UNSUPPORTED;
  if (!gy || !x || !gweight || !workspace || !dims_ok(n, h, w)) return MDE_ERR_INVALID_ARG;
  if (!supported(cin, cout, kWgrad)) return MDE_ERR_UNSUPPORTED;
  hipStream_t s = (hipStream_t)stream;
  const float* xi = (const float*)x;
  const float* g = (const float*)gy;
  float* ws = (float*)workspace;
  const double bytes = 4.0 * n * h * w * (double)(cin + cout);
  if (wide(cin, cout) || wide_pad(cin, cout))
    return launch_wgrad_wide(xi, g, gweight, n, cin, cout, h, w, ws, s);
  if (cin == 3 && cout == 16) return launch_wgrad<3, 16, 8, 4>(xi, g, gweight, n, h, w, ws, bytes, s);
  if (cin == 3 && cout == 32) return launch_wgrad<3, 32, 8, 4>(xi, g, gweight, n, h, w, ws, bytes, s);
  if (cin == 3) return launch_wgrad<3, 64, 4, 4>(xi, g, gweight, n, h, w, ws, bytes, s);
  if (cin == 16 && variant() == 1) return launch_wgrad<16, 16, 8, 4>(xi, g, gweight, n, h, w, ws, bytes, s);
  if (cin == 16 && variant() == 2) return launch_wgrad<16, 16, 4, 2>(xi, g, gweight, n, h, w, ws, bytes, s);
  if (cin == 16) return launch_wgrad<16, 16, 4, 4>(xi, g, gweight, n, h, w, ws, bytes, s);
  if (c32_wide(w)) return launch_wgrad_c32(xi, g, gweight, n, h, w, ws, s);
  if (variant() == 1) return launch_wgrad<32, 32, 4, 2>(xi, g, gweight, n, h, w, ws, bytes, s);
  if (variant() == 2) return launch_wgrad<32, 32, 4, 1>(xi, g, gweight, n, h, w, ws, bytes, s);
  return launch_wgrad<32, 32, 2, 2>(xi, g, gweight, n, h, w, ws, bytes, s);
}


int mde_conv3x3s2_supported(int64_t cin, int64_t cout, int dtype) {
  return dtype == MDE_F32 && (s2_supported(cin, cout) || wide(cin, cout)) ? 1 : 0;
}

size_t mde_conv3x3s2_wgrad_workspace(int64_t n, int64_t cin, int64_t cout, int64_t h, int64_t w,
                                     int dtype) {
  if (dtype != MDE_F32 || !s2_dims_ok(n, h, w)) return 0;
  if (wide(cin, cout)) {
    WidePlan wp;
    return wide_s2_plan(n, cin, cout, h, w, &wp) ? wide_workspace(wp) : 0;
  }
  if (!s2_supported(cin, cout)) return 0;
  if (c32_s2(cin, cout, w)) return c32_s2_workspace(n, h, w);
  const S2Plan p = cin == 3 ? s2_plan<3, 32>(n, h, w) : s2_plan<32, 32>(n, h, w);
  return wgrad_ws_bytes(1, p.grid, p.m);
}

int mde_conv3x3s2_wgrad(const void* gy, const void* x, float* gweight, int64_t n, int64_t cin,
                        int64_t cout, int64_t h, int64_t w, void* workspace, int dtype,
                        void* stream) {
  if (dtype != MDE_F32) return MDE_ERR_UNSUPPORTED;
  if (!gy || !x || !gweight || !workspace || !s2_dims_ok(n, h, w)) return MDE_ERR_INVALID_ARG;
  hipStream_t s = (hipStream_t)stream;
  if (wide(cin, cout))
    return launch_wgrad_wide_s2((const float*)x, (const float*)gy, gweight, n, cin, cout, h, w,
                                (float*)workspace, s);
  if (!s2_supported(cin, cout)) return MDE_ERR_UNSUPPORTED;
  if (c32_s2(cin, cout, w))
    return launch_wgrad_c32_s2((const float*)x, (const float*)gy, gweight, n, h, w,
                               (float*)workspace, s);
  if (cin == 3)
    return launch_wgrad_s2<3, 32>((const float*)x, (const float*)gy, gweight, n, h, w,
                                  (float*)workspace, s);
  return launch_wgrad_s2<32, 32>((const float*)x, (const float*)gy, gweight, n, h, w,
                                 (float*)workspace, s);
}

}
```

monocular_depth_estimation_amd/functional.py:

```python
from __future__ import annotations

import math
from typing import Optional, Sequence

import numpy as np
import torch

from . import _abi

_amp_fwd = torch.amp.custom_fwd(device_type="cuda", cast_inputs=torch.float32)
_amp_bwd = torch.amp.custom_bwd(device_type="cuda")
_bn_fwd = torch.amp.custom_fwd(device_type="cuda")

__all__ = [
    "interpolate", "bilinear_resize", "nearest_resize", "nearest_pyramid", "se_cat", "skip_reduce",
    "minmax", "depth_norm", "ssim3_l1", "depth_loss",
]


def _gpu(*ts):
    for t in ts:
        if t is not None and not t.is_cuda:
            raise RuntimeError(
                "monocular_depth_estimation_amd ops run only on ROCm device tensors "
                f"(got a {t.device} tensor); there is no CPU fallback")


def _ws(nbytes: int, like: torch.Tensor) -> torch.Tensor:
    return torch.empty(max(int(nbytes), 16), dtype=torch.uint8, device=like.device)


def _out_size_and_scales(x: torch.Tensor, size, scale_factor, recompute_scale_factor):
    hi, wi = int(x.shape[-2]), int(x.shape[-1])
    if size is not None:
        if scale_factor is not None:
            raise ValueError("only one of size or scale_factor should be defined")
        if isinstance(size, int):
            size = (size, size)
        ho, wo = int(size[0]), int(size[1])
        scales = (None, None)
    elif scale_factor is not None:
        if isinstance(scale_factor, (int, float)):
            scale_factor = (float(scale_factor), float(scale_factor))
        sf = [float(s) for s in scale_factor]
        ho, wo = int(math.floor(hi * sf[0])), int(math.floor(wi * sf[1]))
        scales = (None, None) if recompute_scale_factor else (sf[0], sf[1])
    else:
        raise ValueError("either size or scale_factor should be defined")

    def one(inp, out, sf):
        if sf is not None and sf > 0:
            return float(np.float32(1.0 / sf))
        return float(np.float32(inp) / np.float32(out))

    return ho, wo, one(hi, ho, scales[0]), one(wi, wo, scales[1])


def _align_scale(inp: int, out: int) -> float:
    if out > 1:
        return float(np.float32(inp - 1) / np.float32(out - 1))
    return 0.0


class GradSlot:

    __slots__ = ("grad",)

    def __init__(self):
        self.grad = None

    def put(self, g):
        self.grad = g if self.grad is None else self.grad + g

    def take(self):
        g, self.grad = self.grad, None
        return g


class _Bilinear(torch.autograd.Function):
    @staticmethod
    @_bn_fwd
    def forward(ctx, x, ho, wo, sh, sw, align, slot=None):
        keep = x.dtype == torch.bfloat16
        x = (x if keep else x.float()).contiguous()
        n, c, hi, wi = x.shape
        y = torch.empty((n, c, ho, wo), dtype=x.dtype, device=x.device)
        _abi.call("mde_bilinear_fwd", _abi.ptr(x), _abi.ptr(y), n, c, hi, wi, ho, wo,
                  sh, sw, int(align), _abi.dtype_code(x), _abi.stream_of(x))
        ctx.meta = (n, c, hi, wi, ho, wo, sh, sw, int(align))
        ctx.slot, ctx.dt = slot, x.dtype
        return y

    @staticmethod
    @_amp_bwd
    def backward(ctx, gy):
        n, c, hi, wi, ho, wo, sh, sw, align = ctx.meta
        gy = gy.to(ctx.dt).contiguous()
        gx = torch.empty((n, c, hi, wi), dtype=gy.dtype, device=gy.device)
        g2 = ctx.slot.take() if ctx.slot is not None else None
        if g2 is not None:
            g2 = g2.to(gy.dtype).contiguous()
            _abi.call("mde_bilinear_bwd2", _abi.ptr(gy), _abi.ptr(g2),
                      _abi.ptr(gx), n, c, hi, wi, ho, wo, sh, sw, align, _abi.dtype_code(gy),
                      _abi.stream_of(gy))
        else:
            _abi.call("mde_bilinear_bwd", _abi.ptr(gy), _abi.ptr(gx), n, c, hi, wi, ho, wo,
                      sh, sw, align, _abi.dtype_code(gy), _abi.stream_of(gy))
        return gx, None, None, None, None, None, None


def bilinear_slot(x, ho, wo, sh, sw, align) -> Optional[GradSlot]:
    if (not torch.is_grad_enabled() or not x.requires_grad
            or x.dtype not in (torch.float32, torch.bfloat16)):
        return None
    n, c, hi, wi = x.shape
    ok = _abi.query("mde_bilinear_bwd2_supported", n, c, hi, wi, ho, wo, sh, sw, int(align))
    return GradSlot() if ok else None


class _Nearest(torch.autograd.Function):
    @staticmethod
    @_amp_fwd
    def forward(ctx, x, ho, wo, sh, sw):
        x = x.contiguous()
        n, c, hi, wi = x.shape
        y = torch.empty((n, c, ho, wo), dtype=x.dtype, device=x.device)
        _abi.call("mde_nearest_fwd", _abi.ptr(x), _abi.ptr(y), n, c, hi, wi, ho, wo,
                  sh, sw, _abi.dtype_code(x), _abi.stream_of(x))
        ctx.meta = (n, c, hi, wi, ho, wo, sh, sw)
        return y

    @staticmethod
    @_amp_bwd
    def backward(ctx, gy):
        n, c, hi, wi, ho, wo, sh, sw = ctx.meta
        gy = gy.contiguous()
        gx = torch.empty((n, c, hi, wi), dtype=gy.dtype, device=gy.device)
        _abi.call("mde_nearest_bwd", _abi.ptr(gy), _abi.ptr(gx), n, c, hi, wi, ho, wo,
                  sh, sw, _abi.dtype_code(gy), _abi.stream_of(gy))
        return gx, None, None, None, None


def bilinear_resize(x, size=None, scale_factor=None, align_corners=False,
                    recompute_scale_factor=None):
    _gpu(x)
    if x.dim() != 4:
        raise ValueError("bilinear_resize expects a 4-D NCHW tensor")
    ho, wo, sh, sw = _out_size_and_scales(x, size, scale_factor, recompute_scale_factor)
    if align_corners:
        sh, sw = _align_scale(x.shape[-2], ho), _align_scale(x.shape[-1], wo)
    return _Bilinear.apply(x, ho, wo, sh, sw, bool(align_corners))


def bilinear_resize_x2_slotted(x):
    _gpu(x)
    if x.dim() != 4:
        raise ValueError("bilinear_resize expects a 4-D NCHW tensor")
    ho, wo, sh, sw = _out_size_and_scales(x, None, 2, None)
    slot = bilinear_slot(x, ho, wo, sh, sw, False)
# ... 303 lines not shown
```

monocular_depth_estimation_amd/nn.py:

```python
from __future__ import annotations

import contextlib
import os

import torch
from torch import nn

from . import _abi
from .functional import GradSlot, _amp_bwd, _amp_fwd, _gpu, _ws

_ACTS = {"none": 0, "relu": 1, "hardswish": 2}


_bn_fwd = torch.amp.custom_fwd(device_type="cuda")


class _BatchNormAct(torch.autograd.Function):
    @staticmethod
    @_bn_fwd
    def forward(ctx, x, weight, bias, prebias, residual, running_mean, running_var, nbt,
                training, momentum, eps, act, stats=None, res_slot=None):
        dt = torch.bfloat16 if x.dtype == torch.bfloat16 else torch.float32
        x = x.to(dt).contiguous()
        residual = residual.to(dt).contiguous() if residual is not None else None
        n, c, h, w = x.shape
        y = torch.empty_like(x)
        mean = torch.empty(c, dtype=torch.float32, device=x.device)
        invstd = torch.empty(c, dtype=torch.float32, device=x.device)
        st = _abi.stream_of(x)
        if training and stats is not None:
            ws = _ws(_abi.query("mde_batchnorm_workspace", n, c, h, w), x)
            _abi.call("mde_batchnorm_fwd_train_stats", _abi.ptr(x), _abi.ptr(weight),
                      _abi.ptr(bias), _abi.ptr(prebias), _abi.ptr(running_mean),
                      _abi.ptr(running_var), _abi.ptr(nbt), float(momentum), float(eps),
                      _abi.ptr(residual), _abi.ptr(y), _abi.ptr(mean), _abi.ptr(invstd), n, c, h,
                      w, act, _abi.ptr(stats), stats.shape[1], _abi.ptr(ws), _abi.dtype_code(x), st)
        elif training:
            ws = _ws(_abi.query("mde_batchnorm_workspace", n, c, h, w), x)
            _abi.call("mde_batchnorm_fwd_train", _abi.ptr(x), _abi.ptr(weight), _abi.ptr(bias),
                      _abi.ptr(prebias), _abi.ptr(running_mean), _abi.ptr(running_var),
                      _abi.ptr(nbt), float(momentum), float(eps), _abi.ptr(residual), _abi.ptr(y),
                      _abi.ptr(mean), _abi.ptr(invstd), n, c, h, w, act, _abi.ptr(ws),
                      _abi.dtype_code(x), st)
        else:
            _abi.call("mde_batchnorm_fwd_eval", _abi.ptr(x), _abi.ptr(weight), _abi.ptr(bias),
                      _abi.ptr(prebias), _abi.ptr(running_mean), _abi.ptr(running_var),
                      float(eps), _abi.ptr(residual), _abi.ptr(y), _abi.ptr(mean),
                      _abi.ptr(invstd), n, c, h, w, act, _abi.dtype_code(x), st)
        ctx.save_for_backward(x, weight, bias, residual, mean, invstd)
        ctx.training, ctx.act, ctx.has_prebias = bool(training), act, prebias is not None
        ctx.res_slot = res_slot
        return y

    @staticmethod
    @_amp_bwd
    def backward(ctx, gy):
        x, weight, bias, residual, mean, invstd = ctx.saved_tensors
        gy = gy.to(x.dtype).contiguous()
        n, c, h, w = x.shape
        gx = torch.empty_like(x)
        gw = torch.empty_like(weight) if ctx.needs_input_grad[1] else None
        gb = torch.empty_like(bias) if ctx.needs_input_grad[2] else None
        gpb = torch.empty_like(weight) if (ctx.has_prebias and ctx.needs_input_grad[3]) else None
        want_r = residual is not None and ctx.needs_input_grad[4]
        gr = torch.empty_like(x) if (want_r and ctx.act) else None
        ws = _ws(_abi.query("mde_batchnorm_workspace", n, c, h, w), x)
        _abi.call("mde_batchnorm_bwd", _abi.ptr(gy), _abi.ptr(x), _abi.ptr(residual),
                  _abi.ptr(weight), _abi.ptr(bias), _abi.ptr(mean), _abi.ptr(invstd),
                  int(ctx.training), _abi.ptr(gx), _abi.ptr(gr), _abi.ptr(gw), _abi.ptr(gb),
                  _abi.ptr(gpb), n, c, h, w, ctx.act, _abi.ptr(ws), _abi.dtype_code(gy),
                  _abi.stream_of(gy))
        if want_r and not ctx.act:
            gr = gy
        if want_r and ctx.res_slot is not None:
            ctx.res_slot.put(gr)
            gr = None
        return gx, gw, gb, gpb, gr, None, None, None, None, None, None, None, None, None


def batch_norm_act(x, bn: nn.BatchNorm2d, act: str = "none", residual=None, prebias=None,
                   stats=None, res_slot=None):
    _gpu(x, residual, prebias)
    if bn.weight is None or bn.bias is None:
        raise NotImplementedError("affine=False BatchNorm has no HIP kernel")
    training = bn.training or not bn.track_running_stats
    if training and bn.momentum is None:
        raise NotImplementedError("cumulative-average BatchNorm (momentum=None) has no HIP kernel")
    track = bn.training and bn.track_running_stats
    return _BatchNormAct.apply(
        x, bn.weight, bn.bias, prebias, residual,
        bn.running_mean if (track or not training) else None,
        bn.running_var if (track or not training) else None,
        bn.num_batches_tracked if track else None,
        training, bn.momentum if bn.momentum is not None else 0.0, bn.eps, _ACTS[act],
        stats if training else None, res_slot if residual is not None else None)


class _Pointwise(torch.autograd.Function):
    @staticmethod
    @_amp_fwd
    def forward(ctx, x, weight):
        x = x.contiguous()
        n, cin, h, w = x.shape
        cout = weight.shape[0]
        w2 = weight.reshape(cout, cin).contiguous()
        y = torch.empty((n, cout, h, w), dtype=x.dtype, device=x.device)
        _abi.call("mde_pointwise_fwd", _abi.ptr(x), None, None, _abi.ptr(w2), _abi.ptr(y), n, cin,
                  cout, h, w,
                  _abi.dtype_code(x), _abi.stream_of(x))
        ctx.save_for_backward(x, w2)
        ctx.wshape = weight.shape
        return y

    @staticmethod
    @_amp_bwd
    def backward(ctx, gy):
        x, w2 = ctx.saved_tensors
        gy = gy.contiguous()
        n, cin, h, w = x.shape
        cout = w2.shape[0]
        gx = torch.empty_like(x) if ctx.needs_input_grad[0] else None
        gw = torch.empty_like(w2)
        ws = _ws(_abi.query("mde_pointwise_workspace", n, cin, cout, h, w), x)
        _abi.call("mde_pointwise_bwd", _abi.ptr(gy), _abi.ptr(x), None, None, _abi.ptr(w2), _abi.ptr(gx),
                  _abi.ptr(gw), n, cin, cout, h, w, _abi.ptr(ws), _abi.dtype_code(gy),
                  _abi.stream_of(gy))
        return gx, gw.view(ctx.wshape)


_PW_BN_SUMS_MAX_CIN = 32


class _BNReluPointwise(torch.autograd.Function):

    @staticmethod
    @_bn_fwd
    def forward(ctx, y1, gamma, beta, prebias, running_mean, running_var, nbt, training, momentum,
                eps, w2, stats1=None, want_stats2=False):
        y1 = (y1 if y1.dtype == torch.bfloat16 else y1.float()).contiguous()
        n, c, h, w = y1.shape
        cout = w2.shape[0]
        w2m = w2.reshape(cout, c).contiguous()
        f32 = dict(dtype=torch.float32, device=y1.device)
        scale, shift = torch.empty(c, **f32), torch.empty(c, **f32)
        mean, invstd = torch.empty(c, **f32), torch.empty(c, **f32)
        st = _abi.stream_of(y1)
        ws = _ws(_abi.query("mde_batchnorm_workspace", n, c, h, w), y1) if training else None
        if training and stats1 is not None:
            _abi.call("mde_batchnorm_fwd_coef_stats", _abi.ptr(y1), _abi.ptr(gamma),
                      _abi.ptr(beta), _abi.ptr(prebias), _abi.ptr(running_mean),
                      _abi.ptr(running_var), _abi.ptr(nbt), float(momentum), float(eps),
                      _abi.ptr(scale), _abi.ptr(shift), _abi.ptr(mean), _abi.ptr(invstd), n, c, h,
                      w, _abi.ptr(stats1), stats1.shape[1], _abi.ptr(ws), _abi.dtype_code(y1), st)
        else:
            _abi.call("mde_batchnorm_fwd_coef", _abi.ptr(y1), _abi.ptr(gamma), _abi.ptr(beta),
                      _abi.ptr(prebias), _abi.ptr(running_mean), _abi.ptr(running_var),
                      _abi.ptr(nbt), float(momentum), float(eps), int(training), _abi.ptr(scale),
                      _abi.ptr(shift), _abi.ptr(mean), _abi.ptr(invstd), n, c, h, w, _abi.ptr(ws),
                      _abi.dtype_code(y1), st)
        y2 = torch.empty((n, cout, h, w), dtype=y1.dtype, device=y1.device)
        if want_stats2:
            nb = _abi.query("mde_pointwise_stats_blocks", n, c, cout, h, w)
            stats2 = torch.empty((cout, nb, 4), **f32)
            _abi.call("mde_pointwise_fwd_stats", _abi.ptr(y1), _abi.ptr(scale), _abi.ptr(shift),
                      _abi.ptr(w2m), _abi.ptr(y2), _abi.ptr(stats2), n, c, cout, h, w,
                      _abi.dtype_code(y1), st)
        else:
            stats2 = torch.empty((cout, 0, 4), **f32)
            _abi.call("mde_pointwise_fwd", _abi.ptr(y1), _abi.ptr(scale), _abi.ptr(shift),
                      _abi.ptr(w2m), _abi.ptr(y2), n, c, cout, h, w, _abi.dtype_code(y1), st)
        ctx.save_for_backward(y1, gamma, beta, mean, invstd, scale, shift, w2m)
        ctx.training, ctx.has_prebias, ctx.w2shape = bool(training), prebias is not None, w2.shape
        ctx.set_materialize_grads(False)
        ctx.mark_non_differentiable(stats2)
        return y2, stats2

    @staticmethod
    @_amp_bwd
    def backward(ctx, gy2, _gstats2):
        if gy2 is None:
            return (None, None, None, None, None, None, None, None, None, None, None, None, None)
        y1, gamma, beta, mean, invstd, scale, shift, w2m = ctx.saved_tensors
        gy2 = gy2.to(y1.dtype).contiguous()
        n, c, h, w = y1.shape
        cout = w2m.shape[0]
        st = _abi.stream_of(gy2)
        gz = torch.empty_like(y1)
        gw2 = torch.empty_like(w2m)
        ws = _ws(_abi.query("mde_pointwise_workspace", n, c, cout, h, w), y1)
        gy1 = torch.empty_like(y1) if ctx.needs_input_grad[0] else None
        gg = torch.empty_like(gamma)
        gb = torch.empty_like(beta)
        gpb = torch.empty_like(gamma) if (ctx.has_prebias and ctx.needs_input_grad[3]) else None
        gy1_out = gy1 if gy1 is not None else torch.empty_like(y1)
        if c <= _PW_BN_SUMS_MAX_CIN:
            sums = torch.empty((c, 2), dtype=torch.float32, device=y1.device)
            _abi.call("mde_pointwise_bwd_bn", _abi.ptr(gy2), _abi.ptr(y1), _abi.ptr(scale),
                      _abi.ptr(shift), _abi.ptr(mean), _abi.ptr(w2m), _abi.ptr(gz),
                      _abi.ptr(gw2), _abi.ptr(sums), n, c, cout, h, w, _abi.ptr(ws),
                      _abi.dtype_code(gy2), st)
            _abi.call("mde_batchnorm_bwd_apply", _abi.ptr(gz), _abi.ptr(y1), None,
                      _abi.ptr(gamma), _abi.ptr(beta), _abi.ptr(mean), _abi.ptr(invstd),
                      int(ctx.training), _abi.ptr(sums), _abi.ptr(gy1_out), None, _abi.ptr(gg),
                      _abi.ptr(gb), _abi.ptr(gpb), n, c, h, w, _ACTS["relu"],
                      _abi.dtype_code(gy2), st)
        else:
            _abi.call("mde_pointwise_bwd", _abi.ptr(gy2), _abi.ptr(y1), _abi.ptr(scale),
                      _abi.ptr(shift), _abi.ptr(w2m), _abi.ptr(gz), _abi.ptr(gw2), n, c, cout, h,
                      w, _abi.ptr(ws), _abi.dtype_code(gy2), st)
            ws2 = _ws(_abi.query("mde_batchnorm_workspace", n, c, h, w), y1)
            _abi.call("mde_batchnorm_bwd", _abi.ptr(gz), _abi.ptr(y1), None, _abi.ptr(gamma),
                      _abi.ptr(beta), _abi.ptr(mean), _abi.ptr(invstd), int(ctx.training),
                      _abi.ptr(gy1_out), None, _abi.ptr(gg), _abi.ptr(gb), _abi.ptr(gpb), n, c,
                      h, w, _ACTS["relu"], _abi.ptr(ws2), _abi.dtype_code(gy2), st)
        return (gy1, gg, gb, gpb, None, None, None, None, None, None, gw2.view(ctx.w2shape), None,
                None)


def bn_relu_pointwise(y1, bn: nn.BatchNorm2d, prebias, conv: nn.Conv2d, stats1=None,
                      want_stats2=False):
    _gpu(y1, prebias)
    if bn.weight is None or bn.bias is None:
        raise NotImplementedError("affine=False BatchNorm has no HIP kernel")
    training = bn.training or not bn.track_running_stats
    if training and bn.momentum is None:
        raise NotImplementedError("cumulative-average BatchNorm (momentum=None) has no HIP kernel")
    track = bn.training and bn.track_running_stats
    y2, stats2 = _BNReluPointwise.apply(
        y1, bn.weight, bn.bias, prebias,
        bn.running_mean if (track or not training) else None,
        bn.running_var if (track or not training) else None,
        bn.num_batches_tracked if track else None,
        training, bn.momentum if bn.momentum is not None else 0.0, bn.eps, conv.weight,
        stats1 if training else None, bool(want_stats2))
    return y2, (stats2 if stats2.shape[1] > 0 else None)


class _SeBnCat(torch.autograd.Function):

    @staticmethod
    @_bn_fwd
    def forward(ctx, ya, yb, ga, ba, pba, gb, bb, pbb, w1, w2, meta_a, meta_b, sta, stb):
        dt = torch.bfloat16 if torch.bfloat16 in (ya.dtype, yb.dtype) else torch.float32
        ya, yb = ya.to(dt).contiguous(), yb.to(dt).contiguous()
        w1, w2 = w1.contiguous(), w2.contiguous()
        n, ca, h, w = ya.shape
        cb = yb.shape[1]
        c, cr = ca + cb, w1.shape[0]
        f32 = dict(dtype=torch.float32, device=ya.device)
        scale, shift = torch.empty(c, **f32), torch.empty(c, **f32)
        mean, invstd = torch.empty(c, **f32), torch.empty(c, **f32)
        st = _abi.stream_of(ya)
        for y, g, b, pb, meta, stt, lo, hi in ((ya, ga, ba, pba, meta_a, sta, 0, ca),
                                                (yb, gb, bb, pbb, meta_b, stb, ca, c)):
            rm, rv, nbt, momentum, eps = meta
            cc = hi - lo
            ws = _ws(_abi.query("mde_batchnorm_workspace", n, cc, h, w), y)
            views = [t[lo:hi] for t in (scale, shift, mean, invstd)]
            if stt is not None:
                _abi.call("mde_batchnorm_fwd_coef_stats", _abi.ptr(y), _abi.ptr(g), _abi.ptr(b),
                          _abi.ptr(pb), _abi.ptr(rm), _abi.ptr(rv), _abi.ptr(nbt), float(momentum),
                          float(eps), *[_abi.ptr(v) for v in views], n, cc, h, w, _abi.ptr(stt),
                          stt.shape[1], _abi.ptr(ws), _abi.dtype_code(y), st)
            else:
                _abi.call("mde_batchnorm_fwd_coef", _abi.ptr(y), _abi.ptr(g), _abi.ptr(b),
                          _abi.ptr(pb), _abi.ptr(rm), _abi.ptr(rv), _abi.ptr(nbt), float(momentum),
                          float(eps), 1, *[_abi.ptr(v) for v in views], n, cc, h, w, _abi.ptr(ws),
                          _abi.dtype_code(y), st)
        out = torch.empty((n, c, h, w), dtype=dt, device=ya.device)
        s, hidden, semean = torch.empty((n, c), **f32), torch.empty((n, cr), **f32), torch.empty((n, c), **f32)
        ws = _ws(_abi.query("mde_se_bn_workspace", n, c, cr, h, w), ya)
        _abi.call("mde_se_bn_fwd", _abi.ptr(ya), ca, _abi.ptr(yb), cb, _abi.ptr(scale),
                  _abi.ptr(shift), _abi.ptr(w1), _abi.ptr(w2), cr, _abi.ptr(out), _abi.ptr(s),
                  _abi.ptr(hidden), _abi.ptr(semean), n, h, w, _abi.ptr(ws), _abi.dtype_code(ya), st)
        ctx.save_for_backward(ya, yb, w1, w2, scale, shift, mean, invstd, s, hidden, semean)
        ctx.has_pb = (pba is not None, pbb is not None)
        return out

    @staticmethod
    @_amp_bwd
    def backward(ctx, gout):
        ya, yb, w1, w2, scale, shift, mean, invstd, s, hidden, semean = ctx.saved_tensors
        gout = gout.to(ya.dtype).contiguous()
        n, ca, h, w = ya.shape
        c, cr = ca + yb.shape[1], w1.shape[0]
        gya, gyb = torch.empty_like(ya), torch.empty_like(yb)
        gg, gbt = torch.empty_like(scale), torch.empty_like(scale)
        gw1, gw2 = torch.empty_like(w1), torch.empty_like(w2)
        ws = _ws(_abi.query("mde_se_bn_workspace", n, c, cr, h, w), ya)
        _abi.call("mde_se_bn_bwd", _abi.ptr(gout), _abi.ptr(ya), ca, _abi.ptr(yb), c - ca,
                  _abi.ptr(scale), _abi.ptr(shift), _abi.ptr(mean), _abi.ptr(invstd), 1,
                  _abi.ptr(w1), _abi.ptr(w2), cr, _abi.ptr(s), _abi.ptr(hidden), _abi.ptr(semean),
                  _abi.ptr(gya), _abi.ptr(gyb), _abi.ptr(gg), _abi.ptr(gbt), _abi.ptr(gw1),
                  _abi.ptr(gw2), n, h, w, _abi.ptr(ws), _abi.dtype_code(gout), _abi.stream_of(gout))
        zpa = torch.zeros(ca, dtype=torch.float32, device=ya.device) if ctx.has_pb[0] else None
        zpb = torch.zeros(c - ca, dtype=torch.float32, device=ya.device) if ctx.has_pb[1] else None
        return (gya, gyb, gg[:ca], gbt[:ca], zpa, gg[ca:], gbt[ca:], zpb, gw1, gw2, None, None,
                None, None)


def se_bn_cat(ya, yb, bn_a: nn.BatchNorm2d, bn_b: nn.BatchNorm2d, pb_a, pb_b, w1, w2,
              stats_a=None, stats_b=None):
    _gpu(ya, yb, pb_a, pb_b, w1, w2)
    for bn in (bn_a, bn_b):
        if bn.weight is None or bn.bias is None or bn.momentum is None or not bn.training:
            raise NotImplementedError("se_bn_cat needs affine, momentum, training-mode BatchNorms")

    def meta(bn):
        track = bn.track_running_stats
        return (bn.running_mean if track else None, bn.running_var if track else None,
                bn.num_batches_tracked if track else None, bn.momentum, bn.eps)

    return _SeBnCat.apply(ya, yb, bn_a.weight, bn_a.bias, pb_a, bn_b.weight, bn_b.bias, pb_b,
                          w1, w2, meta(bn_a), meta(bn_b), stats_a, stats_b)


def pointwise_ok(conv: nn.Conv2d, x) -> bool:
    if (conv.kernel_size != (1, 1) or conv.stride != (1, 1) or conv.padding != (0, 0)
            or conv.dilation != (1, 1) or conv.groups != 1 or x.dim() != 4
            or conv.weight.dtype != torch.float32):
        return False
    return bool(_abi.query("mde_pointwise_supported", conv.in_channels, conv.out_channels,
                           x.shape[2], x.shape[3]))


CONV3X3_HIP = {
    (3, 16): (True, True, True),
    (3, 32): (True, True, True),
    (3, 64): (True, True, True),
    (16, 16): (True, True, True),
    (32, 32): (False, False, True),
}
WIDE_WGRAD_ALL = os.environ.get("MDE_WIDE_WGRAD", "1") != "0"
WIDE_PAD = os.environ.get("MDE_WIDE_PAD", "1") != "0"
WINO_MIN_BLOCKS = int(os.environ.get("MDE_WINO_MIN_BLOCKS", "256"))
if WIDE_WGRAD_ALL:
    CONV3X3_HIP.update({(64, 64): (False, False, True), (128, 64): (False, False, True),
                        (128, 128): (False, False, True), (256, 256): (False, False, True)})


class _Conv3x3(torch.autograd.Function):
    @staticmethod
    @_amp_fwd
    def forward(ctx, x, weight, passes, want_stats=False, gx_slot=None):
        wkey = weight
        x = x.contiguous()
        weight = weight.contiguous()
        n, cin, h, w = x.shape
        cout = weight.shape[0]
        stats = torch.empty((cout, 0, 4), dtype=torch.float32, device=x.device)
        ctx.gx_slot = gx_slot
        u_flip = None
        if passes[0] == WINO:
            y = torch.empty((n, cout, h, w), dtype=x.dtype, device=x.device)
            st = _abi.stream_of(x)
            if want_stats:
                nb = _abi.query("mde_wino_stats_blocks", n, cin, cout, h, w)
                stats = torch.empty((cout, nb, 4), dtype=torch.float32, device=x.device)
            flip = passes[1] == WINO
            sc = _ACTIVE_PACK
            ent = sc.wino.get(wkey) if sc is not None else None
            if ent is not None and wkey in sc.wino_packed and (ent[1] is not None or not flip):
                u, u_flip = ent[0], (ent[1] if flip else None)
            else:
                ub = _abi.query("mde_wino_weight_bytes", cin, cout) // 4
                u = torch.empty(ub, dtype=torch.float32, device=x.device)
                if flip:
                    u_flip = torch.empty(ub, dtype=torch.float32, device=x.device)
                    _abi.call("mde_wino_weight2", _abi.ptr(weight), _abi.ptr(u), _abi.ptr(u_flip),
                              cin, cout, st)
                else:
                    _abi.call("mde_wino_weight", _abi.ptr(weight), _abi.ptr(u), cin, cout, 0, st)
                if (sc is not None and ent is None and isinstance(wkey, nn.Parameter)
                        and not torch.cuda.is_current_stream_capturing()):
                    sc.wino[wkey] = (u, u_flip, cin, cout)
            _abi.call("mde_wino_conv_stats", _abi.ptr(x), _abi.ptr(u), _abi.ptr(y),
                      _abi.ptr(stats) if want_stats else None, n, cin, cout, h, w, 0,
                      _abi.dtype_code(x), st)
        elif passes[0] == WIDE:
            y = torch.empty((n, cout, h, w), dtype=x.dtype, device=x.device)
            _abi.call("mde_conv3x3_wide_fwd", _abi.ptr(x), _abi.ptr(weight), _abi.ptr(y), n, cin,
                      cout, h, w, _abi.dtype_code(x), _abi.stream_of(x))
        elif passes[0]:
            y = torch.empty((n, cout, h, w), dtype=x.dtype, device=x.device)
            if want_stats:
                nb = _abi.query("mde_conv3x3_stats_blocks", n, cin, cout, h, w, _abi.MDE_F32)
                stats = torch.empty((cout, nb, 4), dtype=torch.float32, device=x.device)
                _abi.call("mde_conv3x3_fwd_stats", _abi.ptr(x), _abi.ptr(weight), _abi.ptr(y),
                          _abi.ptr(stats), n, cin, cout, h, w, _abi.dtype_code(x),
                          _abi.stream_of(x))
            else:
                _abi.call("mde_conv3x3_fwd", _abi.ptr(x), _abi.ptr(weight), _abi.ptr(y), n, cin,
                          cout, h, w, _abi.dtype_code(x), _abi.stream_of(x))
        else:
            y = torch.nn.functional.conv2d(x, weight, None, 1, 1)
        ctx.save_for_backward(x, weight)
        ctx.passes = passes
        ctx.u_flip = u_flip
        ctx.set_materialize_grads(False)
        ctx.mark_non_differentiable(stats)
        return y, stats

    @staticmethod
    @_amp_bwd
    def backward(ctx, gy, _gstats):
        g2 = ctx.gx_slot.take() if ctx.gx_slot is not None else None
        if gy is None:
            return (g2, None, None, None, None)
        x, weight = ctx.saved_tensors
        gy = gy.contiguous()
        n, cin, h, w = x.shape
        cout = weight.shape[0]
        gx = gw = None
        st = _abi.stream_of(gy)
        if ctx.needs_input_grad[0]:
            if ctx.passes[1] == WINO:
                gx = torch.empty_like(x)
                u = ctx.u_flip
                if u is None:
                    u = torch.empty(_abi.query("mde_wino_weight_bytes", cin, cout) // 4,
                                    dtype=torch.float32, device=x.device)
                    _abi.call("mde_wino_weight", _abi.ptr(weight), _abi.ptr(u), cin, cout, 1, st)
                if g2 is not None and g2.dtype == gy.dtype == torch.float32:
                    g2 = g2.contiguous()
                    _abi.call("mde_wino_conv_acc", _abi.ptr(gy), _abi.ptr(u), _abi.ptr(g2),
                              _abi.ptr(gx), n, cout, cin, h, w, 1, _abi.dtype_code(gy), st)
                    g2 = None
                else:
                    _abi.call("mde_wino_conv", _abi.ptr(gy), _abi.ptr(u), _abi.ptr(gx), n, cout,
                              cin, h, w, 1, _abi.dtype_code(gy), st)
            elif ctx.passes[1] == WIDE:
                gx = torch.empty_like(x)
                _abi.call("mde_conv3x3_wide_bwd_data", _abi.ptr(gy), _abi.ptr(weight), _abi.ptr(gx),
                          n, cin, cout, h, w, _abi.dtype_code(gy), st)
            elif ctx.passes[1]:
                gx = torch.empty_like(x)
                _abi.call("mde_conv3x3_bwd_data", _abi.ptr(gy), _abi.ptr(weight), _abi.ptr(gx), n,
                          cin, cout, h, w, _abi.dtype_code(gy), st)
            else:
                gx = torch.ops.aten.convolution_backward(
                    gy, x, weight, None, (1, 1), (1, 1), (1, 1), False, (0, 0), 1,
                    (True, False, False))[0]
        if ctx.needs_input_grad[1]:
            if ctx.passes[2]:
                gw = torch.empty_like(weight)
                ws = _ws(_abi.query("mde_conv3x3_wgrad_workspace", n, cin, cout, h, w,
                                    _abi.MDE_F32), x)
                _abi.call("mde_conv3x3_wgrad", _abi.ptr(gy), _abi.ptr(x), _abi.ptr(gw), n, cin,
                          cout, h, w, _abi.ptr(ws), _abi.dtype_code(gy), st)
            else:
                gw = torch.ops.aten.convolution_backward(
                    gy, x, weight, None, (1, 1), (1, 1), (1, 1), False, (0, 0), 1,
                    (False, True, False))[1]
        if g2 is not None:
            gx = g2 if gx is None else gx + g2
        return gx, gw, None, None, None


CONV3X3_HIP_BF16 = {
    (16, 16): (True, True, True),
    (32, 32): (True, True, True),
}
if os.environ.get("MDE_C3BF32", "1") == "0":
    del CONV3X3_HIP_BF16[(32, 32)]


def _autocast_bf16(x) -> bool:
    return (x.is_cuda and torch.is_autocast_enabled("cuda")
            and torch.get_autocast_dtype("cuda") == torch.bfloat16)


def _conv3x3_bf16_path(cin: int, cout: int, x, weight) -> bool:
    return ((_autocast_bf16(x) or x.dtype == torch.bfloat16)
            and weight.dtype == torch.float32
            and (cin, cout) in CONV3X3_HIP_BF16 and x.shape[-1] % 4 == 0)


class _Conv3x3Bf16(torch.autograd.Function):

    @staticmethod
    @_bn_fwd
    def forward(ctx, x, weight, passes, want_stats=False):
        x = x.contiguous()
        weight = weight.contiguous()
        n, cin, h, w = x.shape
        cout = weight.shape[0]
        bf = _abi.MDE_BF16
        stats = torch.empty((cout, 0, 4), dtype=torch.float32, device=x.device)
        if passes[0]:
            y = torch.empty((n, cout, h, w), dtype=torch.bfloat16, device=x.device)
            if want_stats:
                nb = _abi.query("mde_conv3x3_stats_blocks", n, cin, cout, h, w, bf)
                stats = torch.empty((cout, nb, 4), dtype=torch.float32, device=x.device)
                _abi.call("mde_conv3x3_fwd_stats", _abi.ptr(x), _abi.ptr(weight), _abi.ptr(y),
                          _abi.ptr(stats), n, cin, cout, h, w, bf, _abi.stream_of(x))
            else:
                _abi.call("mde_conv3x3_fwd", _abi.ptr(x), _abi.ptr(weight), _abi.ptr(y), n, cin,
                          cout, h, w, bf, _abi.stream_of(x))
        else:
            y = torch.nn.functional.conv2d(x, weight.to(torch.bfloat16), None, 1, 1)
        ctx.save_for_backward(x, weight)
        ctx.passes = passes
        ctx.set_materialize_grads(False)
        ctx.mark_non_differentiable(stats)
        return y, stats

    @staticmethod
    @_amp_bwd
    def backward(ctx, gy, _gstats):
        if gy is None:
            return (None, None, None, None)
        x, weight = ctx.saved_tensors
        gy = gy.to(torch.bfloat16).contiguous()
        n, cin, h, w = x.shape
        cout = weight.shape[0]
        bf = _abi.MDE_BF16
        gx = gw = None
        st = _abi.stream_of(gy)
        if ctx.needs_input_grad[0]:
            if ctx.passes[1]:
                gx = torch.empty_like(x)
                _abi.call("mde_conv3x3_bwd_data", _abi.ptr(gy), _abi.ptr(weight), _abi.ptr(gx), n,
                          cin, cout, h, w, bf, st)
            else:
                gx = torch.ops.aten.convolution_backward(
                    gy, x, weight.to(torch.bfloat16), None, (1, 1), (1, 1), (1, 1), False, (0, 0),
                    1, (True, False, False))[0]
        if ctx.needs_input_grad[1]:
            if ctx.passes[2]:
                gw = torch.empty_like(weight)
                ws = _ws(_abi.query("mde_conv3x3_wgrad_workspace", n, cin, cout, h, w, bf), x)
                _abi.call("mde_conv3x3_wgrad", _abi.ptr(gy), _abi.ptr(x), _abi.ptr(gw), n, cin,
                          cout, h, w, _abi.ptr(ws), bf, st)
            else:
                gw = torch.ops.aten.convolution_backward(
                    gy, x, weight.to(torch.bfloat16), None, (1, 1), (1, 1), (1, 1), False, (0, 0),
                    1, (False, True, False))[1].float()
        return gx, gw, None, None

# ... 363 lines not shown
            and x.numel() < (1 << 31)
            and bool(_abi.query("mde_stem_bf16_supported", 3, conv.out_channels, x.shape[2],
                                x.shape[3])))


CONVBF = os.environ.get("MDE_CONVBF", "1") != "0"
_CONVBF_OK: dict = {}


def convbf_ok(conv: nn.Conv2d, x) -> bool:
    if not (CONVBF and x.is_cuda and x.dim() == 4
            and (_autocast_bf16(x) or x.dtype == torch.bfloat16)
            and conv.weight.dtype == torch.float32 and conv.groups == 1
            and conv.dilation == (1, 1) and conv.padding_mode == "zeros"
            and conv.stride in ((1, 1), (2, 2))
            and ((conv.kernel_size == (3, 3) and conv.padding == (1, 1))
                 or (conv.kernel_size == (1, 1) and conv.padding == (0, 0)))):
        return False
    key = (x.shape[0], conv.in_channels, conv.out_channels, x.shape[2], x.shape[3],
           conv.kernel_size[0], conv.stride[0])
    ok = _CONVBF_OK.get(key)
    if ok is None:
        ok = all(_abi.query("mde_convbf_supported_n", *key, p) for p in (0, 1, 2))
        _CONVBF_OK[key] = ok
    return ok


def conv_bf16(conv: nn.Conv2d, x):
    _gpu(x)
    return _ConvBf16.apply(x, conv.weight, conv.kernel_size[0], conv.stride[0], False)[0]


def conv_bf16_stats(conv: nn.Conv2d, x):
    _gpu(x)
    y, stats = _ConvBf16.apply(x, conv.weight, conv.kernel_size[0], conv.stride[0], True)
    return y, (stats if stats.shape[1] > 0 else None)


class _GuideConvBf16(torch.autograd.Function):

    @staticmethod
    def forward(ctx, x, weight, want_stats):
        x = x.contiguous()
        weight = weight.contiguous()
        n, _, h, w = x.shape
        cout = weight.shape[0]
        y = torch.empty((n, cout, h, w), dtype=torch.bfloat16, device=x.device)
        nb = _abi.query("mde_conv3x3_guide_bf16_stats_blocks", n, cout, h, w) if want_stats else 0
        stats = torch.empty((cout, nb, 4), dtype=torch.float32, device=x.device)
        _abi.call("mde_conv3x3_guide_bf16_fwd", _abi.ptr(x), _abi.ptr(weight), _abi.ptr(y),
                  _abi.ptr(stats) if nb else None, n, cout, h, w, _abi.stream_of(x))
        ctx.save_for_backward(x, weight)
        ctx.set_materialize_grads(False)
        ctx.mark_non_differentiable(stats)
        return y, stats

    @staticmethod
    def backward(ctx, gy, _gstats):
        if gy is None:
            return (None, None, None)
        x, weight = ctx.saved_tensors
        gw = None
        if ctx.needs_input_grad[1]:
            n, cin, h, w = x.shape
            cout = weight.shape[0]
            gw = torch.empty_like(weight)
            if gy.dtype == torch.bfloat16 and w % 4 == 0:
                gy = gy.contiguous()
                ws = _ws(_abi.query("mde_conv3x3_guide_bf16_wgrad_workspace", n, cout, h, w), x)
                _abi.call("mde_conv3x3_guide_bf16_wgrad", _abi.ptr(gy), _abi.ptr(x), _abi.ptr(gw),
                          n, cout, h, w, _abi.ptr(ws), _abi.stream_of(gy))
            else:
                gyf = gy.float().contiguous()
                ws = _ws(_abi.query("mde_conv3x3_wgrad_workspace", n, cin, cout, h, w,
                                    _abi.MDE_F32), x)
                _abi.call("mde_conv3x3_wgrad", _abi.ptr(gyf), _abi.ptr(x), _abi.ptr(gw), n, cin,
                          cout, h, w, _abi.ptr(ws), _abi.MDE_F32, _abi.stream_of(gyf))
        return None, gw, None


GUIDE_BF16 = os.environ.get("MDE_GUIDE_BF16", "1") != "0"


def _conv3x3_apply(x, weight, passes, want_stats, gx_slot=None):
    if weight.dtype != torch.float32:
        raise TypeError(f"conv3x3: the HIP kernels take a float32 weight, got {weight.dtype}")
    cin, cout = x.shape[1], weight.shape[0]
    if (GUIDE_BF16 and cin == 3 and cout in (16, 32, 64) and passes[0] and x.dtype == torch.float32
            and _autocast_bf16(x) and not x.requires_grad
            and x.numel() < (1 << 31)):
        return _GuideConvBf16.apply(x, weight, bool(want_stats))
    if _conv3x3_bf16_path(cin, cout, x, weight):
        return _Conv3x3Bf16.apply(x.to(torch.bfloat16), weight, tuple(passes), want_stats)
    return _Conv3x3.apply(x, weight, tuple(passes), want_stats, gx_slot)


def conv3x3(x, weight, passes=(True, True, True), gx_slot=None):
    _gpu(x)
    return _conv3x3_apply(x, weight, passes, False, gx_slot)[0]


def conv3x3_stats(x, weight, passes=(True, True, True), gx_slot=None):
    _gpu(x)
    y, stats = _conv3x3_apply(x, weight, passes, bool(passes[0]), gx_slot)
    return y, (stats if stats.shape[1] > 0 else None)


def conv_bn(conv: nn.Conv2d, bn: "BatchNorm2d", x, residual=None):
    passes = conv3x3_passes(conv, x) if x.is_cuda else None
    want = bn.training or not bn.track_running_stats
    st = None
    if pointwise_ok(conv, x):
        _gpu(x)
        y = _Pointwise.apply(x, conv.weight)
    elif passes is not None:
        if want and passes[0] and _epilogue_stats_pay("conv3x3", conv, x):
            y, st = conv3x3_stats(x, conv.weight, passes)
        else:
            y = conv3x3(x, conv.weight, passes)
    elif stem_ok(conv, x):
        y = _StemBf16.apply(x, conv.weight)
    elif convbf_ok(conv, x):
        if want and _epilogue_stats_pay("convbf", conv, x):
            y, st = conv_bf16_stats(conv, x)
        else:
            y = conv_bf16(conv, x)
    elif conv3x3s2_ok(conv, x):
        y = _Conv3x3S2.apply(x, conv.weight)
    elif conv1x1_ok(conv, x):
        y = _Conv1x1.apply(x, conv.weight, conv.stride[0])
    else:
        y = torch.nn.functional.conv2d(x, conv.weight, None, conv.stride, conv.padding,
                                       conv.dilation, conv.groups)
    return batch_norm_act(y, bn, bn.act, residual, conv.bias, st)


_STATS_ROUTE: dict = {}


def _epilogue_stats_pay(kind, conv, x) -> bool:
    n, cin, h, w = x.shape
    k, s = conv.kernel_size[0], conv.stride[0]
    key = (kind, n, cin, conv.out_channels, h, w, k, s, x.dtype)
    hit = _STATS_ROUTE.get(key)
    if hit is None:
        cout, pad = conv.out_channels, k // 2
        ho, wo = (h + 2 * pad - k) // s + 1, (w + 2 * pad - k) // s + 1
        if kind == "convbf":
            nb = _abi.query("mde_convbf_stats_blocks", n, cin, cout, h, w, k, s)
            dt = _abi.MDE_BF16
        else:
            dt = _abi.MDE_BF16 if (x.dtype == torch.bfloat16 or _autocast_bf16(x)) else _abi.MDE_F32
            nb = _abi.query("mde_conv3x3_stats_blocks", n, cin, cout, h, w, dt)
        hit = nb > 0 and _abi.query("mde_batchnorm_stats_route", n, cout, ho, wo, nb, dt) == 1
        _STATS_ROUTE[key] = hit
    return hit


def conv_nobias_stats(conv: nn.Conv2d, x, bn: nn.BatchNorm2d, gx_slot=None):
    if x.is_cuda and (bn.training or not bn.track_running_stats):
        passes = conv3x3_passes(conv, x)
        if passes is not None:
            if passes[0] and _epilogue_stats_pay("conv3x3", conv, x):
                return conv3x3_stats(x, conv.weight, passes, gx_slot)
        elif convbf_ok(conv, x) and _epilogue_stats_pay("convbf", conv, x):
            return conv_bf16_stats(conv, x)
    return conv_nobias(conv, x, gx_slot), None


RESIDUAL_SLOT = os.environ.get("MDE_RES_SLOT", "1") != "0"


def residual_grad_slot(conv: nn.Conv2d, x):
    if not (RESIDUAL_SLOT and torch.is_grad_enabled() and x.is_cuda and x.requires_grad
            and x.dtype == torch.float32 and not _autocast_bf16(x)):
        return None
    passes = conv3x3_passes(conv, x)
    if passes is None or passes[1] != WINO:
        return None
    return GradSlot()


def conv_nobias(conv: nn.Conv2d, x, gx_slot=None):
    passes = conv3x3_passes(conv, x) if x.is_cuda else None
    if passes is not None:
        return conv3x3(x, conv.weight, passes, gx_slot)
    if gx_slot is not None:
# ... 57 lines not shown
            and x.dim() == 4 and conv.out_channels == 1 and conv.bias is not None
            and conv.kernel_size == (3, 3) and conv.stride == (1, 1) and conv.padding == (1, 1)
            and conv.dilation == (1, 1) and conv.groups == 1
            and conv.weight.dtype == torch.float32
            and bool(_abi.query("mde_head_conv_supported", x.shape[0], x.shape[1], x.shape[2],
                                x.shape[3])))


class _HeadConv(torch.autograd.Function):

    @staticmethod
    def forward(ctx, x, weight, bias):
        x = x.contiguous()
        n, c, h, w = x.shape
        wt = weight.contiguous()
        y = torch.empty((n, 1, h, w), dtype=torch.float32, device=x.device)
        _abi.call("mde_head_conv_fwd", _abi.ptr(x), _abi.ptr(wt), _abi.ptr(bias), _abi.ptr(y), n, c,
                  h, w, 0, _abi.stream_of(x))
        ctx.save_for_backward(x, wt)
        return y

    @staticmethod
    def backward(ctx, gy):
        x, wt = ctx.saved_tensors
        n, c, h, w = x.shape
        gy = gy.contiguous()
        st = _abi.stream_of(gy)
        gx = gw = gb = None
        if ctx.needs_input_grad[0]:
            gx = torch.empty_like(x)
            _abi.call("mde_head_conv_dgrad", _abi.ptr(gy), _abi.ptr(wt), _abi.ptr(gx), n, c, h, w, 0,
                      st)
        if ctx.needs_input_grad[1]:
            gw = torch.empty_like(wt)
            ws = _ws(_abi.query("mde_head_conv_wgrad_workspace", n, c, h, w), gy)
            _abi.call("mde_head_conv_wgrad", _abi.ptr(gy), _abi.ptr(x), _abi.ptr(gw), n, c, h, w,
                      _abi.ptr(ws), 0, st)
        if ctx.needs_input_grad[2]:
            gb = torch.empty(1, dtype=torch.float32, device=gy.device)
            ws = _ws(_abi.query("mde_chansum_workspace", n, 1, h * w), gy)
            _abi.call("mde_chansum", _abi.ptr(gy), _abi.ptr(gb), n, 1, h * w, _abi.ptr(ws), 0, st)
        return gx, gw, gb


class Conv2d(nn.Conv2d):

    def forward(self, x):
        if x.is_cuda and self.padding_mode == "zeros":
            if self.bias is None:
                return conv_nobias(self, x)
            passes = conv3x3_passes(self, x)
            if passes is not None and (passes[0] or passes[1]):
                y = conv3x3(x, self.weight, passes)
                if CHANSUM and y.dtype == torch.float32 and _abi.query(
                        "mde_chansum_workspace", y.shape[0], y.shape[1], y.shape[2] * y.shape[3]):
                    return _BiasAdd.apply(y, self.bias)
                return y + self.bias.to(y.dtype).view(1, -1, 1, 1)
            if convbf_ok(self, x):
                y = conv_bf16(self, x)
                return y + self.bias.to(y.dtype).view(1, -1, 1, 1)
            if head_conv_ok(self, x):
                return _HeadConv.apply(x, self.weight, self.bias)
            if CHANSUM and conv1x1_ok(self, x):
                y = _Conv1x1.apply(x, self.weight, self.stride[0])
                if _abi.query("mde_chansum_workspace", y.shape[0], y.shape[1],
                              y.shape[2] * y.shape[3]):
                    return _BiasAdd.apply(y, self.bias)
                return y + self.bias.view(1, -1, 1, 1)
        return super().forward(x)


def _bnrelu_pw_at(mods, i, x_shape) -> bool:
    if i + 4 >= len(mods):
        return False
    c0, b0, r0, c1, b1 = mods[i:i + 5]
    return (isinstance(c0, nn.Conv2d) and c0.bias is not None and c0.padding_mode == "zeros"
            and isinstance(b0, BatchNorm2d) and b0.act == "relu"
            and isinstance(r0, nn.Identity)
            and isinstance(c1, nn.Conv2d) and c1.bias is not None and isinstance(b1, BatchNorm2d)
            and c1.kernel_size == (1, 1) and c1.stride == (1, 1) and c1.padding == (0, 0)
            and c1.groups == 1 and c1.in_channels == c0.out_channels)


def run_sequential(seq: nn.Sequential, x):
    mods = list(seq)
    i = 0
    while i < len(mods):
        m = mods[i]
        if x.is_cuda and _bnrelu_pw_at(mods, i, x.shape):
            want = mods[i + 1].training or not mods[i + 1].track_running_stats
            passes = conv3x3_passes(m, x)
            if passes is not None and want:
                y1, st1 = conv3x3_stats(x, m.weight, passes)
            else:
                y1, st1 = conv_nobias(m, x), None
            if pointwise_ok(mods[i + 3], y1):
                b2 = mods[i + 4]
                y2, st2 = bn_relu_pointwise(y1, mods[i + 1], m.bias, mods[i + 3], st1,
                                            b2.training or not b2.track_running_stats)
                x = batch_norm_act(y2, b2, b2.act, None, mods[i + 3].bias, st2)
                i += 5
                continue
            x = batch_norm_act(y1, mods[i + 1], mods[i + 1].act, None, m.bias, st1)
            i += 2
            continue
        if (isinstance(m, nn.Conv2d) and m.bias is not None and i + 1 < len(mods)
                and isinstance(mods[i + 1], BatchNorm2d) and m.padding_mode == "zeros"):
            x = conv_bn(m, mods[i + 1], x)
            i += 2
        elif (isinstance(m, Conv2d) and m.bias is None and i + 1 < len(mods)
              and isinstance(mods[i + 1], BatchNorm2d) and m.padding_mode == "zeros"):
            y, st = conv_nobias_stats(m, x, mods[i + 1])
            x = mods[i + 1](y, stats=st)
            i += 2
        else:
            x = m(x)
            i += 1
    return x


def run_sequential_raw(seq: nn.Sequential, x):
    mods = list(seq)
    if (len(mods) != 6 or not x.is_cuda or x.dtype not in (torch.float32, torch.bfloat16)
            or not _bnrelu_pw_at(mods, 0, x.shape)
            or not isinstance(mods[5], nn.Identity) or mods[4].act != "relu"
            or not mods[1].training or not mods[4].training):
        return None
    m, c1 = mods[0], mods[3]
    k = m.kernel_size
    same = (m.stride == (1, 1) and m.dilation == (1, 1) and k[0] % 2 == 1 and k[1] % 2 == 1
            and m.padding == (k[0] // 2, k[1] // 2))
    passes = conv3x3_passes(m, x)
    if passes is not None:
        y1, st1 = conv3x3_stats(x, m.weight, passes)
    else:
        y1, st1 = conv_nobias(m, x), None
    if same and pointwise_ok(c1, x):
        y2, st2 = bn_relu_pointwise(y1, mods[1], m.bias, c1, st1, True)
        return y2, st2, mods[4], c1.bias
    x1 = batch_norm_act(y1, mods[1], "relu", None, m.bias, st1)
    y2 = torch.nn.functional.conv2d(x1, c1.weight, None, c1.stride, c1.padding, c1.dilation,
                                    c1.groups)
    return y2, None, mods[4], c1.bias


class _SkipReduceBN(torch.autograd.Function):

    @staticmethod
    @_bn_fwd
    def forward(ctx, r, d, weight, bias, gamma, beta, prebias, meta, stats, d_slot=None):
        dt = torch.bfloat16 if r.dtype == torch.bfloat16 else torch.float32
        r, d = r.to(dt).contiguous(), d.to(dt).contiguous()
        n, cin, h, w = r.shape
        cout = weight.shape[0]
        wm = weight.reshape(cout, cin).contiguous()
        f32 = dict(dtype=torch.float32, device=r.device)
        scale, shift = torch.empty(cin, **f32), torch.empty(cin, **f32)
        mean, invstd = torch.empty(cin, **f32), torch.empty(cin, **f32)
        rm, rv, nbt, momentum, eps = meta
        st = _abi.stream_of(r)
        ws = _ws(_abi.query("mde_batchnorm_workspace", n, cin, h, w), r)
        if stats is not None:
            _abi.call("mde_batchnorm_fwd_coef_stats", _abi.ptr(r), _abi.ptr(gamma), _abi.ptr(beta),
                      _abi.ptr(prebias), _abi.ptr(rm), _abi.ptr(rv), _abi.ptr(nbt), float(momentum),
                      float(eps), _abi.ptr(scale), _abi.ptr(shift), _abi.ptr(mean), _abi.ptr(invstd),
                      n, cin, h, w, _abi.ptr(stats), stats.shape[1], _abi.ptr(ws),
                      _abi.dtype_code(r), st)
        else:
            _abi.call("mde_batchnorm_fwd_coef", _abi.ptr(r), _abi.ptr(gamma), _abi.ptr(beta),
                      _abi.ptr(prebias), _abi.ptr(rm), _abi.ptr(rv), _abi.ptr(nbt), float(momentum),
                      float(eps), 1, _abi.ptr(scale), _abi.ptr(shift), _abi.ptr(mean),
                      _abi.ptr(invstd), n, cin, h, w, _abi.ptr(ws), _abi.dtype_code(r), st)
        out = torch.empty((n, cout, h, w), dtype=dt, device=r.device)
        _abi.call("mde_skip_reduce_bn_fwd", _abi.ptr(r), _abi.ptr(d), _abi.ptr(scale),
                  _abi.ptr(shift), _abi.ptr(wm), _abi.ptr(bias), _abi.ptr(out), n, cin, cout, h, w,
                  _abi.dtype_code(r), st)
        ctx.save_for_backward(r, d, wm, gamma, beta, scale, shift, mean, invstd)
        ctx.wshape, ctx.has_pb, ctx.d_slot = weight.shape, prebias is not None, d_slot
        return out

    @staticmethod
    @_amp_bwd
    def backward(ctx, gout):
        r, d, wm, gamma, beta, scale, shift, mean, invstd = ctx.saved_tensors
        gout = gout.to(r.dtype).contiguous()
        n, cin, h, w = r.shape
        cout = wm.shape[0]
        st = _abi.stream_of(gout)
        gs = torch.empty_like(r)
        gw, gb = torch.empty_like(wm), torch.empty(cout, dtype=torch.float32, device=r.device)
        use_sums = bool(_abi.query("mde_skip_reduce_bn_supported", cin, cout, h, w, 1))
        sums = torch.empty((cin, 2), dtype=torch.float32, device=r.device) if use_sums else None
        ws = _ws(_abi.query("mde_skip_reduce_bn_workspace", n, cin, cout, h, w), r)
        _abi.call("mde_skip_reduce_bn_bwd", _abi.ptr(gout), _abi.ptr(r), _abi.ptr(d),
                  _abi.ptr(scale), _abi.ptr(shift), _abi.ptr(mean), _abi.ptr(wm), _abi.ptr(gs),
                  _abi.ptr(gw), _abi.ptr(gb), _abi.ptr(sums), n, cin, cout, h, w, _abi.ptr(ws),
                  _abi.dtype_code(gout), st)
        gr = torch.empty_like(r)
        gg, gbeta = torch.empty_like(gamma), torch.empty_like(beta)
        gpb = torch.empty_like(gamma) if (ctx.has_pb and ctx.needs_input_grad[6]) else None
        if sums is not None:
            _abi.call("mde_batchnorm_bwd_apply", _abi.ptr(gs), _abi.ptr(r), None, _abi.ptr(gamma),
                      _abi.ptr(beta), _abi.ptr(mean), _abi.ptr(invstd), 1, _abi.ptr(sums),
                      _abi.ptr(gr), None, _abi.ptr(gg), _abi.ptr(gbeta), _abi.ptr(gpb), n, cin, h,
                      w, _ACTS["relu"], _abi.dtype_code(gout), st)
        else:
            ws2 = _ws(_abi.query("mde_batchnorm_workspace", n, cin, h, w), r)
            _abi.call("mde_batchnorm_bwd", _abi.ptr(gs), _abi.ptr(r), None, _abi.ptr(gamma),
                      _abi.ptr(beta), _abi.ptr(mean), _abi.ptr(invstd), 1, _abi.ptr(gr), None,
                      _abi.ptr(gg), _abi.ptr(gbeta), _abi.ptr(gpb), n, cin, h, w, _ACTS["relu"],
                      _abi.ptr(ws2), _abi.dtype_code(gout), st)
        if ctx.d_slot is not None and ctx.needs_input_grad[1]:
            ctx.d_slot.put(gs)
            gd = None
        else:
            gd = gs
        return gr, gd, gw.view(ctx.wshape), gb, gg, gbeta, gpb, None, None, None


def skip_reduce_bn_ok(r, cout: int) -> bool:
    return (r.dim() == 4 and r.dtype in (torch.float32, torch.bfloat16) and
# ... 129 lines not shown
```

Baseline: 1003 images/s.

## Fold BN+ReLU backward into conv3x3 dgrad and wgrad operand loads

Adds a per-channel BN backward coefficient kernel, plus conv3x3 data-gradient and weight-gradient kernel variants that apply the BN+ReLU backward transform on the fly while loading the gradient tile from gz and the saved pre-BN output y1. A slot object passes y1 and the coefficients from the fused BN-ReLU-pointwise backward to the conv backward, so the full-size BN input gradient is never written and read back. This applies only to small-channel guided-upsampling shapes in fp32. In exchange the conv loads read an extra tensor, the kernels gain register pressure, and the autograd state is coupled through a side channel.

```diff
diff --git a/include/mde_abi.h b/include/mde_abi.h
--- a/include/mde_abi.h
+++ b/include/mde_abi.h
@@ -170,6 +170,10 @@
                             void* gresidual, float* ggamma, float* gbeta, float* gprebias,
                             int64_t n, int64_t c, int64_t h, int64_t w, int act, int dtype,
                             void* stream);
+int mde_batchnorm_bwd_coef(const float* gamma, const float* beta, const float* mean,
+                           const float* invstd, int training, const float* sums, float* coef,
+                           float* ggamma, float* gbeta, float* gprebias, int64_t n, int64_t c,
+                           int64_t h, int64_t w, void* stream);
 
 size_t mde_window_attn_workspace(int64_t b, int64_t h, int64_t w, int64_t c,
                                  int64_t heads, int64_t window);
@@ -241,6 +245,12 @@
 int mde_conv3x3_wgrad(const void* gy, const void* x, float* gweight, int64_t n, int64_t cin,
                       int64_t cout, int64_t h, int64_t w, void* workspace, int dtype,
                       void* stream);
+int mde_conv3x3_bwd_data_bn(const void* gz, const void* y1, const float* coef,
+                            const float* weight, void* gx, int64_t n, int64_t cin, int64_t cout,
+                            int64_t h, int64_t w, int dtype, void* stream);
+int mde_conv3x3_wgrad_bn(const void* gz, const void* y1, const float* coef, const void* x,
+                         float* gweight, int64_t n, int64_t cin, int64_t cout, int64_t h,
+                         int64_t w, void* workspace, int dtype, void* stream);
 
 int mde_conv3x3s2_supported(int64_t cin, int64_t cout, int dtype);
 size_t mde_conv3x3s2_wgrad_workspace(int64_t n, int64_t cin, int64_t cout, int64_t h, int64_t w,
diff --git a/monocular_depth_estimation_amd/_abi.py b/monocular_depth_estimation_amd/_abi.py
--- a/monocular_depth_estimation_amd/_abi.py
+++ b/monocular_depth_estimation_amd/_abi.py
@@ -104,6 +104,12 @@
     "mde_conv3x3_bwd_data": (_int, [_vp, _vp, _vp, _i64, _i64, _i64, _i64, _i64, _int, _vp]),
     "mde_conv3x3_wgrad_workspace": (_sz, [_i64, _i64, _i64, _i64, _i64, _int]),
     "mde_conv3x3_wgrad": (_int, [_vp, _vp, _vp, _i64, _i64, _i64, _i64, _i64, _vp, _int, _vp]),
+    "mde_conv3x3_bwd_data_bn": (_int, [_vp, _vp, _vp, _vp, _vp, _i64, _i64, _i64, _i64, _i64, _int,
+                                       _vp]),
+    "mde_conv3x3_wgrad_bn": (_int, [_vp, _vp, _vp, _vp, _vp, _i64, _i64, _i64, _i64, _i64, _vp,
+                                    _int, _vp]),
+    "mde_batchnorm_bwd_coef": (_int, [_vp, _vp, _vp, _vp, _int, _vp, _vp, _vp, _vp, _vp, _i64,
+                                      _i64, _i64, _i64, _vp]),
     "mde_conv3x3s2_supported": (_int, [_i64, _i64, _int]),
     "mde_conv3x3s2_wgrad_workspace": (_sz, [_i64, _i64, _i64, _i64, _i64, _int]),
     "mde_conv3x3s2_wgrad": (_int, [_vp, _vp, _vp, _i64, _i64, _i64, _i64, _i64, _vp, _int, _vp]),
diff --git a/monocular_depth_estimation_amd/csrc/bn.hip b/monocular_depth_estimation_amd/csrc/bn.hip
--- a/monocular_depth_estimation_amd/csrc/bn.hip
+++ b/monocular_depth_estimation_amd/csrc/bn.hip
@@ -517,6 +517,17 @@
   }
 }
 
+__global__ void __launch_bounds__(64) bn_bwd_coef_kernel(float* __restrict__ coef, BwdArgs P) {
+  const int64_t ch = blockIdx.x;
+  double a, b;
+  wave_slices(P.part, ch, P.slices, &a, &b);
+  if (threadIdx.x == 0) {
+    const BwdCh k = bwd_channel(P, ch, a, b, true);
+    float* o = coef + 5 * ch;
+    o[0] = k.sc; o[1] = k.sh; o[2] = k.A; o[3] = k.B; o[4] = k.D;
+  }
+}
+
 template <typename T>
 __global__ void __launch_bounds__(256)
     bn_bwd_apply_table_kernel(const T* __restrict__ gy, const T* __restrict__ x,
@@ -1143,4 +1154,17 @@
              : bwd_apply<float>(gy, x, residual, gx, gresidual, n, c, hw, act, P, s);
 }
 
-}
+int mde_batchnorm_bwd_coef(const float* gamma, const float* beta, const float* mean,
+                           const float* invstd, int training, const float* sums, float* coef,
+                           float* ggamma, float* gbeta, float* gprebias, int64_t n, int64_t c,
+                           int64_t h, int64_t w, void* stream) {
+  if (!gamma || !beta || !mean || !invstd || !sums || !coef || !args_ok(n, c, h, w))
+    return MDE_ERR_INVALID_ARG;
+  hipStream_t s = (hipStream_t)stream;
+  BwdArgs P{gamma, beta, mean, invstd, sums, 1, n * h * w, training, ggamma, gbeta, gprebias};
+  MDE_LAUNCH(mde::K_BN_BWD_FINAL, 4.0 * (double)c * (2 + 4 + 5 + 3), s, bn_bwd_coef_kernel,
+             dim3((unsigned)c), dim3(64), 0, coef, P);
+  return MDE_OK;
+}
+
+}
diff --git a/monocular_depth_estimation_amd/csrc/conv3x3.hip b/monocular_depth_estimation_amd/csrc/conv3x3.hip
--- a/monocular_depth_estimation_amd/csrc/conv3x3.hip
+++ b/monocular_depth_estimation_amd/csrc/conv3x3.hip
@@ -1,4 +1,5 @@
 #include <cstdlib>
+#include <type_traits>
 
 #include "common.h"
 
@@ -146,6 +147,156 @@
   }
 };
 
+struct BnCoef {
+  float sc, sh, A, B, D;
+};
+
+__device__ __forceinline__ BnCoef bn_coef(const float* __restrict__ coef, int c) {
+  const float* p = coef + 5 * c;
+  return {p[0], p[1], p[2], p[3], p[4]};
+}
+
+template <int SEQ>
+__device__ __forceinline__ float bn_fold(float g, float y, const BnCoef& k) {
+#pragma clang fp contract(off)
+  const float e = __builtin_fmaf(y, k.sc, k.sh) > 0.f ? g : 0.f;
+  const float ae = k.A * e;
+  float t;
+  if constexpr (SEQ == 1) {
+    t = __builtin_fmaf(k.B, y, ae);
+  } else {
+    const float by = k.B * y;
+    t = ae + by;
+  }
+  return t + k.D;
+}
+
+template <int CI, int CIP, int XR, int SEQ>
+struct HaloTileBn {
+  using H = HaloTile<CI, CIP, XR>;
+  H g;
+  BnCoef hk[H::NH];
+
+  __device__ __forceinline__ void init(const float* __restrict__ coef, int lane, int wvu) {
+#pragma unroll
+    for (int q = 0; q < H::NH; ++q) {
+      const int e = 64 * q + lane;
+      const int ri = wvu + 4 * (e >> 1);
+      const int c = ri / XR;
+      hk[q] = bn_coef(coef, e < 2 * H::RPWV && ri < H::ROWS && c < CI ? c : 0);
+    }
+  }
+
+  __device__ __forceinline__ void load(const float* __restrict__ gi, int h, int w, int r0, int c0,
+                                       int lane, int wvu) {
+    g.load(gi, h, w, r0, c0, lane, wvu);
+  }
+
+  template <int PS>
+  __device__ __forceinline__ void store(float* sx, const float* __restrict__ coef,
+                                        const float* __restrict__ yi, int h, int w, int r0,
+                                        int c0, int lane, int wvu) const {
+    H y;
+    y.load(yi, h, w, r0, c0, lane, wvu);
+#pragma unroll
+    for (int k = 0; k < H::RPWV; ++k) {
+      const int ri = wvu + 4 * k;
+      if (H::ROWS % 4 == 0 || ri < H::ROWS) {
+        const int c = ri / XR;
+        const BnCoef kf = bn_coef(coef, c < CI ? c : 0);
+        const float v = bn_fold<SEQ>(g.a[k], y.a[k], kf);
+        sx[c * PS + (ri % XR) * kXW + lane] = (g.am >> k) & 1 ? v : 0.f;
+      }
+    }
+#pragma unroll
+    for (int q = 0; q < H::NH; ++q) {
+      const int e = 64 * q + lane;
+      const int ri = wvu + 4 * (e >> 1);
+      if (e < 2 * H::RPWV && ri < H::ROWS) {
+        const float v = bn_fold<SEQ>(g.b[q], y.b[q], hk[q]);
+        sx[(ri / XR) * PS + (ri % XR) * kXW + 64 + (e & 1)] = (g.bm >> q) & 1u ? v : 0.f;
+      }
+    }
+  }
+};
+
+template <int CO, int TH, bool FULL, int SEQ>
+struct GradTileBn {
+  static constexpr int ROWS = CO * TH;
+  static constexpr int PER = ROWS / 16;
+  static_assert(ROWS % 16 == 0 && TH % 4 == 0 && PER <= 16, "uniform channel, mask width");
+  static constexpr bool LATE = PER >= 16;
+  float4 g[PER], y[LATE ? 1 : PER];
+  uint64_t vm;
+
+  __device__ __forceinline__ static unsigned geo(int i, int h, int w, int r0, int c0, int lane,
+                                                 int wvu, unsigned (&a)[4]) {
+    const int gc = c0 + 4 * (lane & 15);
+    const int ri = 16 * i + 4 * wvu + (lane >> 4);
+    const int c = ri / TH, gr = r0 + ri % TH;
+    const bool rok = gr < h;
+    const unsigned row = (unsigned)((c * h + gr) * w + gc);
+    if (FULL || (w & 3) == 0) {
+      const bool ok = rok && (FULL || gc < w);
+      a[0] = ok ? row : 0u;
+      return ok ? 0xfu : 0u;
+    }
+    unsigned m = 0;
+#pragma unroll
+    for (int j = 0; j < 4; ++j) {
+      const bool ok = rok && gc + j < w;
+      a[j] = ok ? row + j : 0u;
+      m |= ok ? 1u << j : 0u;
+    }
+    return m;
+  }
+
+  __device__ __forceinline__ static float4 ld(const float* __restrict__ p, int w,
+                                              const unsigned (&a)[4]) {
+    if (FULL || (w & 3) == 0) return *reinterpret_cast<const float4*>(p + a[0]);
+    return make_float4(p[a[0]], p[a[1]], p[a[2]], p[a[3]]);
+  }
+
+  __device__ __forceinline__ void load(const float* __restrict__ gi, const float* __restrict__ yi,
+                                       int h, int w, int r0, int c0, int lane, int wvu) {
+    vm = 0;
+#pragma unroll
+    for (int i = 0; i < PER; ++i) {
+      unsigned a[4];
+      const unsigned m = geo(i, h, w, r0, c0, lane, wvu, a);
+      g[i] = ld(gi, w, a);
+      if constexpr (!LATE) y[i] = ld(yi, w, a);
+      vm |= (uint64_t)m << (4 * i);
+    }
+  }
+
+  template <int PSG>
+  __device__ __forceinline__ void store(float* sg, const float* __restrict__ coef,
+                                        const float* __restrict__ yi, int h, int w, int r0,
+                                        int c0, int lane, int wvu) const {
+#pragma unroll
+    for (int i = 0; i < PER; ++i) {
+      const int ri = 16 * i + 4 * wvu + (lane >> 4);
+      const BnCoef kf = bn_coef(coef, (16 * i + 4 * wvu) / TH);
+      const unsigned m = (unsigned)(vm >> (4 * i));
+      float4 v;
+      if constexpr (LATE) {
+        unsigned a[4];
+        (void)geo(i, h, w, r0, c0, lane, wvu, a);
+        v = ld(yi, w, a);
+      } else {
+        v = y[i];
+      }
+      float4 t;
+      t.x = m & 1u ? bn_fold<SEQ>(g[i].x, v.x, kf) : 0.f;
+      t.y = m & 2u ? bn_fold<SEQ>(g[i].y, v.y, kf) : 0.f;
+      t.z = m & 4u ? bn_fold<SEQ>(g[i].z, v.z, kf) : 0.f;
+      t.w = m & 8u ? bn_fold<SEQ>(g[i].w, v.w, kf) : 0.f;
+      *reinterpret_cast<float4*>(sg + (ri / TH) * PSG + (ri % TH) * kTW + 4 * (lane & 15)) = t;
+    }
+  }
+};
+
 struct TileGeo {
   int img, r0, c0;
 };
@@ -167,13 +318,17 @@
   return {tile / tiles_per_img, (t / tiles_w) * th, (t % tiles_w) * kTW};
 }
 
-template <int CI, int CO, int RPW, bool FLIP, bool STATS = false, typename TO = float>
+template <int CI, int CO, int RPW, bool FLIP, bool STATS = false, typename TO = float,
+          int FOLD = 0>
 __global__ void __launch_bounds__(256, 2)
     conv3x3_fwd_kernel(const float* __restrict__ x, const float* __restrict__ wt,
                        TO* __restrict__ y, int h, int w, int tiles_w, int tiles_per_img,
-                       int ntiles, float* __restrict__ stats = nullptr) {
+                       int ntiles, float* __restrict__ stats = nullptr,
+                       const float* __restrict__ y1 = nullptr,
+                       const float* __restrict__ coef = nullptr) {
   static_assert(!(STATS && FLIP), "statistics are a forward epilogue");
   constexpr bool RB = sizeof(TO) == 2;
+  static_assert(!FOLD || (FLIP && !RB), "the folded operand is a data gradient's");
   constexpr int CIP = cpad4(CI);
   constexpr int TH = 4 * RPW;
   constexpr int XR = TH + 2;
@@ -220,23 +375,24 @@
 #pragma unroll
   for (int nb = 0; nb < (STATS ? NB : 1); ++nb) run[nb] = {0.f, 0.f, 0.f, 0.f};
   bool first = true;
-  HaloTile<CI, CIP, XR> T;
+  std::conditional_t<FOLD != 0, HaloTileBn<CI, CIP, XR, FOLD>, HaloTile<CI, CIP, XR>> T;
+  if constexpr (FOLD != 0) T.init(coef, lane, wvu);
+  auto load = [&](const TileGeo& t) {
+    T.load(x + t.img * img_in, h, w, t.r0, t.c0, lane, wvu);
+  };
   const TileWalk tw = tile_walk(ntiles);
   int tile = tw.t0;
-  if (tile < tw.end) {
-    const TileGeo g = tile_geo(tile, TH, tiles_w, tiles_per_img);
-    T.load(x + g.img * img_in, h, w, g.r0, g.c0, lane, wvu);
-  }
+  if (tile < tw.end) load(tile_geo(tile, TH, tiles_w, tiles_per_img));
   for (; tile < tw.end; tile += tw.step) {
     const TileGeo g = tile_geo(tile, TH, tiles_w, tiles_per_img);
     __syncthreads();
-    T.template store<PS, RB>(sx, lane, wvu);
+    if constexpr (FOLD != 0)
+      T.template store<PS>(sx, coef, y1 + g.img * img_in, h, w, g.r0, g.c0, lane, wvu);
+    else
+      T.template store<PS, RB>(sx, lane, wvu);
     __syncthreads();
     const int nxt = tile + tw.step;
-    if (nxt < tw.end) {
-      const TileGeo gn = tile_geo(nxt, TH, tiles_w, tiles_per_img);
-      T.load(x + gn.img * img_in, h, w, gn.r0, gn.c0, lane, wvu);
-    }
+    if (nxt < tw.end) load(tile_geo(nxt, TH, tiles_w, tiles_per_img));
 
     f4 acc[RPW][4][NB];
 #pragma unroll
@@ -425,11 +581,12 @@
   static constexpr int M = CO * NP;
 };
 
-template <int CI, int CO, int TH, int PW, bool FULL>
+template <int CI, int CO, int TH, int PW, bool FULL, int FOLD = 0>
 __global__ void __launch_bounds__(256, 2)
     conv3x3_wgrad_kernel(const float* __restrict__ x, const float* __restrict__ gy,
                          float* __restrict__ part, int h, int w, int tiles_w,
-                         int tiles_per_img, int ntiles) {
+                         int tiles_per_img, int ntiles, const float* __restrict__ y1 = nullptr,
+                         const float* __restrict__ coef = nullptr) {
   using C = WgradCfg<CI, CO, TH, PW>;
   __shared__ float smem[C::SMEM];
   float* sx = smem;
@@ -462,25 +619,29 @@
 
   for (int e = tid; e < C::XR * kXW; e += 256) smem[C::ZERO + e] = 0.f;
   HaloTile<CI, C::CIP, C::XR> T;
-  GradTile<CO, TH, FULL> G;
+  std::conditional_t<FOLD != 0, GradTileBn<CO, TH, FULL, FOLD>, GradTile<CO, TH, FULL>> G;
+  auto load = [&](const TileGeo& t) {
+    if constexpr (FOLD != 0)
+      G.load(gy + t.img * img_out, y1 + t.img * img_out, h, w, t.r0, t.c0, lane, wvu);
+    else
+      G.load(gy + t.img * img_out, h, w, t.r0, t.c0, lane, wvu);
+    T.load(x + t.img * img_in, h, w, t.r0, t.c0, lane, wvu);
+  };
   const TileWalk tw = tile_walk(ntiles);
   int tile = tw.t0;
-  if (tile < tw.end) {
-    const TileGeo g = tile_geo(tile, TH, tiles_w, tiles_per_img);
-    G.load(gy + g.img * img_out, h, w, g.r0, g.c0, lane, wvu);
-    T.load(x + g.img * img_in, h, w, g.r0, g.c0, lane, wvu);
-  }
+  if (tile < tw.end) load(tile_geo(tile, TH, tiles_w, tiles_per_img));
   for (; tile < tw.end; tile += tw.step) {
     __syncthreads();
     T.template store<C::PSX>(sx, lane, wvu);
-    G.template store<C::PSG>(sg, lane, wvu);
+    if constexpr (FOLD != 0) {
+      const TileGeo g = tile_geo(tile, TH, tiles_w, tiles_per_img);
+      G.template store<C::PSG>(sg, coef, y1 + g.img * img_out, h, w, g.r0, g.c0, lane, wvu);
+    } else {
+      G.template store<C::PSG>(sg, lane, wvu);
+    }
     __syncthreads();
     const int nxt = tile + tw.step;
-    if (nxt < tw.end) {
-      const TileGeo gn = tile_geo(nxt, TH, tiles_w, tiles_per_img);
-      G.load(gy + gn.img * img_out, h, w, gn.r0, gn.c0, lane, wvu);
-      T.load(x + gn.img * img_in, h, w, gn.r0, gn.c0, lane, wvu);
-    }
+    if (nxt < tw.end) load(tile_geo(nxt, TH, tiles_w, tiles_per_img));
 
     for (int rr = 0; rr < C::RPWG; ++rr) {
       const int row = pg * C::RPWG + rr;
@@ -1994,6 +2155,24 @@
   return MDE_OK;
 }
 
+template <int C, int RPW, int SEQ>
+int launch_dgrad_bn(const float* gz, const float* y1, const float* coef, const float* wt,
+                    float* out, int64_t n, int64_t h, int64_t w, hipStream_t s) {
+  constexpr auto kernel = conv3x3_fwd_kernel<C, C, RPW, true, false, float, SEQ>;
+  const double flops = 2.0 * 9 * C * C * (double)(n * h * w);
+  const double bytes = 4.0 * n * h * w * (double)(3 * C);
+  constexpr int TH = 4 * RPW;
+  const int tiles_w = (int)mde::cdiv(w, kTW);
+  const int tiles_per_img = (int)(mde::cdiv(h, TH) * tiles_w);
+  const int64_t nt = n * tiles_per_img;
+  if (nt > 0x7fffffff) return MDE_ERR_INVALID_ARG;
+  const int res = resident_blocks<kernel>();
+  MDE_LAUNCH_MFMA(mde::K_C3_DGRAD, bytes, flops, s, kernel, dim3(nt < res ? (int)nt : res),
+                  dim3(256), 0, gz, wt, out, (int)h, (int)w, tiles_w, tiles_per_img, (int)nt,
+                  (float*)nullptr, y1, coef);
+  return MDE_OK;
+}
+
 struct WgradPlan {
   int th, tiles_w, tiles_per_img, ntiles, grid, m, np, cip;
 };
@@ -2042,6 +2221,35 @@
   return launch_reduce(ws, gw, 1, p.grid, p.m, ReduceMap{0, p.np, p.cip, CI, CO}, s);
 }
 
+template <int CI, int CO, int TH, int PW, int SEQ>
+int launch_wgrad_bn(const float* x, const float* gz, const float* y1, const float* coef,
+                    float* gw, int64_t n, int64_t h, int64_t w, float* ws, hipStream_t s) {
+  const WgradPlan p = wgrad_plan<CI, CO, TH, PW>(n, h, w);
+  const double flops = 2.0 * 9 * CI * CO * (double)(n * h * w);
+  const double bytes = 4.0 * n * h * w * (double)(CI + 2 * CO);
+  bool full = false;
+  if constexpr (SEQ == 1) {
+    full = w % kTW == 0;
+    if (full && CI == 3)
+      MDE_LAUNCH(mde::K_C3_WGRAD_GUIDE, bytes, s,
+                 (conv3x3_wgrad_kernel<CI, CO, TH, PW, true, SEQ>), dim3(p.grid), dim3(256), 0, x,
+                 gz, ws, (int)h, (int)w, p.tiles_w, p.tiles_per_img, p.ntiles, y1, coef);
+    else if (full)
+      MDE_LAUNCH_MFMA(mde::K_C3_WGRAD, bytes, flops, s,
+                      (conv3x3_wgrad_kernel<CI, CO, TH, PW, true, SEQ>), dim3(p.grid), dim3(256),
+                      0, x, gz, ws, (int)h, (int)w, p.tiles_w, p.tiles_per_img, p.ntiles, y1, coef);
+  }
+  if (!full && CI == 3)
+    MDE_LAUNCH(mde::K_C3_WGRAD_GUIDE, bytes, s,
+               (conv3x3_wgrad_kernel<CI, CO, TH, PW, false, SEQ>), dim3(p.grid), dim3(256), 0, x,
+               gz, ws, (int)h, (int)w, p.tiles_w, p.tiles_per_img, p.ntiles, y1, coef);
+  else if (!full)
+    MDE_LAUNCH_MFMA(mde::K_C3_WGRAD, bytes, flops, s,
+                    (conv3x3_wgrad_kernel<CI, CO, TH, PW, false, SEQ>), dim3(p.grid), dim3(256), 0,
+                    x, gz, ws, (int)h, (int)w, p.tiles_w, p.tiles_per_img, p.ntiles, y1, coef);
+  return launch_reduce(ws, gw, 1, p.grid, p.m, ReduceMap{0, p.np, p.cip, CI, CO}, s);
+}
+
 struct S2Plan {
   int ho, wo, tiles_w, tiles_per_img, ntiles, grid, m, np, cip;
 };
@@ -2427,6 +2635,41 @@
   return launch_wgrad<32, 32, 2, 2>(xi, g, gweight, n, h, w, ws, bytes, s);
 }
 
+int mde_conv3x3_bwd_data_bn(const void* gz, const void* y1, const float* coef,
+                            const float* weight, void* gx, int64_t n, int64_t cin, int64_t cout,
+                            int64_t h, int64_t w, int dtype, void* stream) {
+  if (dtype != MDE_F32) return MDE_ERR_UNSUPPORTED;
+  if (!gz || !y1 || !coef || !weight || !gx || !dims_ok(n, h, w)) return MDE_ERR_INVALID_ARG;
+  if (cin != 16 || cout != 16) return MDE_ERR_UNSUPPORTED;
+  hipStream_t s = (hipStream_t)stream;
+  const float* g = (const float*)gz;
+  const float* y = (const float*)y1;
+  if ((h * w) % 4 == 0) return launch_dgrad_bn<16, 1, 1>(g, y, coef, weight, (float*)gx, n, h, w, s);
+  return launch_dgrad_bn<16, 1, 2>(g, y, coef, weight, (float*)gx, n, h, w, s);
+}
+
+int mde_conv3x3_wgrad_bn(const void* gz, const void* y1, const float* coef, const void* x,
+                         float* gweight, int64_t n, int64_t cin, int64_t cout, int64_t h,
+                         int64_t w, void* workspace, int dtype, void* stream) {
+  if (dtype != MDE_F32) return MDE_ERR_UNSUPPORTED;
+  if (!gz || !y1 || !coef || !x || !gweight || !workspace || !dims_ok(n, h, w))
+    return MDE_ERR_INVALID_ARG;
+  hipStream_t s = (hipStream_t)stream;
+  const float* xi = (const float*)x;
+  const float* g = (const float*)gz;
+  const float* y = (const float*)y1;
+  float* ws = (float*)workspace;
+  const bool v4 = (h * w) % 4 == 0;
+#define MDE_WG(CI, CO, TH)                                                              \
+  (v4 ? launch_wgrad_bn<CI, CO, TH, 4, 1>(xi, g, y, coef, gweight, n, h, w, ws, s)     \
+      : launch_wgrad_bn<CI, CO, TH, 4, 2>(xi, g, y, coef, gweight, n, h, w, ws, s))
+  if (cin == 3 && cout == 16) return MDE_WG(3, 16, 8);
+  if (cin == 3 && cout == 32) return MDE_WG(3, 32, 8);
+  if (cin == 16 && cout == 16) return MDE_WG(16, 16, 4);
+#undef MDE_WG
+  return MDE_ERR_UNSUPPORTED;
+}
+
 
 int mde_conv3x3s2_supported(int64_t cin, int64_t cout, int dtype) {
   return dtype == MDE_F32 && (s2_supported(cin, cout) || wide(cin, cout)) ? 1 : 0;
diff --git a/monocular_depth_estimation_amd/functional.py b/monocular_depth_estimation_amd/functional.py
--- a/monocular_depth_estimation_amd/functional.py
+++ b/monocular_depth_estimation_amd/functional.py
@@ -75,6 +75,22 @@
     def take(self):
         g, self.grad = self.grad, None
         return g
+
+
+class BnFoldSlot:
+
+    __slots__ = ("y1", "coef")
+
+    def __init__(self):
+        self.y1 = self.coef = None
+
+    def put(self, y1, coef):
+        self.y1, self.coef = y1, coef
+
+    def take(self):
+        r = (self.y1, self.coef) if self.coef is not None else None
+        self.y1 = self.coef = None
+        return r
 
 
 class _Bilinear(torch.autograd.Function):
diff --git a/monocular_depth_estimation_amd/nn.py b/monocular_depth_estimation_amd/nn.py
--- a/monocular_depth_estimation_amd/nn.py
+++ b/monocular_depth_estimation_amd/nn.py
@@ -7,7 +7,7 @@
 from torch import nn
 
 from . import _abi
-from .functional import GradSlot, _amp_bwd, _amp_fwd, _gpu, _ws
+from .functional import BnFoldSlot, GradSlot, _amp_bwd, _amp_fwd, _gpu, _ws
 
 _ACTS = {"none": 0, "relu": 1, "hardswish": 2}
 
@@ -136,7 +136,7 @@
     @staticmethod
     @_bn_fwd
     def forward(ctx, y1, gamma, beta, prebias, running_mean, running_var, nbt, training, momentum,
-                eps, w2, stats1=None, want_stats2=False):
+                eps, w2, stats1=None, want_stats2=False, bn_slot=None):
         y1 = (y1 if y1.dtype == torch.bfloat16 else y1.float()).contiguous()
         n, c, h, w = y1.shape
         cout = w2.shape[0]
@@ -171,6 +171,7 @@
                       _abi.ptr(w2m), _abi.ptr(y2), n, c, cout, h, w, _abi.dtype_code(y1), st)
         ctx.save_for_backward(y1, gamma, beta, mean, invstd, scale, shift, w2m)
         ctx.training, ctx.has_prebias, ctx.w2shape = bool(training), prebias is not None, w2.shape
+        ctx.bn_slot = bn_slot
         ctx.set_materialize_grads(False)
         ctx.mark_non_differentiable(stats2)
         return y2, stats2
@@ -179,7 +180,7 @@
     @_amp_bwd
     def backward(ctx, gy2, _gstats2):
         if gy2 is None:
-            return (None, None, None, None, None, None, None, None, None, None, None, None, None)
+            return (None,) * 14
         y1, gamma, beta, mean, invstd, scale, shift, w2m = ctx.saved_tensors
         gy2 = gy2.to(y1.dtype).contiguous()
         n, c, h, w = y1.shape
@@ -188,10 +189,25 @@
         gz = torch.empty_like(y1)
         gw2 = torch.empty_like(w2m)
         ws = _ws(_abi.query("mde_pointwise_workspace", n, c, cout, h, w), y1)
-        gy1 = torch.empty_like(y1) if ctx.needs_input_grad[0] else None
+        fold = (ctx.bn_slot is not None and ctx.needs_input_grad[0]
+                and c <= _PW_BN_SUMS_MAX_CIN and y1.dtype == torch.float32)
+        gy1 = torch.empty_like(y1) if (ctx.needs_input_grad[0] and not fold) else None
         gg = torch.empty_like(gamma)
         gb = torch.empty_like(beta)
         gpb = torch.empty_like(gamma) if (ctx.has_prebias and ctx.needs_input_grad[3]) else None
+        if fold:
+            sums = torch.empty((c, 2), dtype=torch.float32, device=y1.device)
+            coef = torch.empty((c, 5), dtype=torch.float32, device=y1.device)
+            _abi.call("mde_pointwise_bwd_bn", _abi.ptr(gy2), _abi.ptr(y1), _abi.ptr(scale),
+                      _abi.ptr(shift), _abi.ptr(mean), _abi.ptr(w2m), _abi.ptr(gz),
+                      _abi.ptr(gw2), _abi.ptr(sums), n, c, cout, h, w, _abi.ptr(ws),
+                      _abi.dtype_code(gy2), st)
+            _abi.call("mde_batchnorm_bwd_coef", _abi.ptr(gamma), _abi.ptr(beta), _abi.ptr(mean),
+                      _abi.ptr(invstd), int(ctx.training), _abi.ptr(sums), _abi.ptr(coef),
+                      _abi.ptr(gg), _abi.ptr(gb), _abi.ptr(gpb), n, c, h, w, st)
+            ctx.bn_slot.put(y1, coef)
+            return (gz, gg, gb, gpb, None, None, None, None, None, None, gw2.view(ctx.w2shape),
+                    None, None, None)
         gy1_out = gy1 if gy1 is not None else torch.empty_like(y1)
         if c <= _PW_BN_SUMS_MAX_CIN:
             sums = torch.empty((c, 2), dtype=torch.float32, device=y1.device)
@@ -214,11 +230,11 @@
                       _abi.ptr(gy1_out), None, _abi.ptr(gg), _abi.ptr(gb), _abi.ptr(gpb), n, c,
                       h, w, _ACTS["relu"], _abi.ptr(ws2), _abi.dtype_code(gy2), st)
         return (gy1, gg, gb, gpb, None, None, None, None, None, None, gw2.view(ctx.w2shape), None,
-                None)
+                None, None)
 
 
 def bn_relu_pointwise(y1, bn: nn.BatchNorm2d, prebias, conv: nn.Conv2d, stats1=None,
-                      want_stats2=False):
+                      want_stats2=False, bn_slot=None):
     _gpu(y1, prebias)
     if bn.weight is None or bn.bias is None:
         raise NotImplementedError("affine=False BatchNorm has no HIP kernel")
@@ -232,7 +248,7 @@
         bn.running_var if (track or not training) else None,
         bn.num_batches_tracked if track else None,
         training, bn.momentum if bn.momentum is not None else 0.0, bn.eps, conv.weight,
-        stats1 if training else None, bool(want_stats2))
+        stats1 if training else None, bool(want_stats2), bn_slot)
     return y2, (stats2 if stats2.shape[1] > 0 else None)
 
 
@@ -342,7 +358,7 @@
 class _Conv3x3(torch.autograd.Function):
     @staticmethod
     @_amp_fwd
-    def forward(ctx, x, weight, passes, want_stats=False, gx_slot=None):
+    def forward(ctx, x, weight, passes, want_stats=False, gx_slot=None, bn_slot=None):
         wkey = weight
         x = x.contiguous()
         weight = weight.contiguous()
@@ -350,6 +366,7 @@
         cout = weight.shape[0]
         stats = torch.empty((cout, 0, 4), dtype=torch.float32, device=x.device)
         ctx.gx_slot = gx_slot
+        ctx.bn_slot = bn_slot
         u_flip = None
         if passes[0] == WINO:
             y = torch.empty((n, cout, h, w), dtype=x.dtype, device=x.device)
@@ -405,14 +422,32 @@
     @_amp_bwd
     def backward(ctx, gy, _gstats):
         g2 = ctx.gx_slot.take() if ctx.gx_slot is not None else None
+        fold = ctx.bn_slot.take() if ctx.bn_slot is not None else None
         if gy is None:
-            return (g2, None, None, None, None)
+            return (g2, None, None, None, None, None)
         x, weight = ctx.saved_tensors
         gy = gy.contiguous()
         n, cin, h, w = x.shape
         cout = weight.shape[0]
         gx = gw = None
         st = _abi.stream_of(gy)
+        if fold is not None:
+            y1, coef = fold
+            if ctx.needs_input_grad[0]:
+                gx = torch.empty_like(x)
+                _abi.call("mde_conv3x3_bwd_data_bn", _abi.ptr(gy), _abi.ptr(y1), _abi.ptr(coef),
+                          _abi.ptr(weight), _abi.ptr(gx), n, cin, cout, h, w,
+                          _abi.dtype_code(gy), st)
+            if ctx.needs_input_grad[1]:
+                gw = torch.empty_like(weight)
+                ws = _ws(_abi.query("mde_conv3x3_wgrad_workspace", n, cin, cout, h, w,
+                                    _abi.MDE_F32), x)
+                _abi.call("mde_conv3x3_wgrad_bn", _abi.ptr(gy), _abi.ptr(y1), _abi.ptr(coef),
+                          _abi.ptr(x), _abi.ptr(gw), n, cin, cout, h, w, _abi.ptr(ws),
+                          _abi.dtype_code(gy), st)
+            if g2 is not None:
+                gx = g2 if gx is None else gx + g2
+            return gx, gw, None, None, None, None
         if ctx.needs_input_grad[0]:
             if ctx.passes[1] == WINO:
                 gx = torch.empty_like(x)
@@ -454,7 +489,7 @@
                     (False, True, False))[1]
         if g2 is not None:
             gx = g2 if gx is None else gx + g2
-        return gx, gw, None, None, None
+        return gx, gw, None, None, None, None
 
 
 CONV3X3_HIP_BF16 = {
@@ -984,10 +1019,12 @@
 GUIDE_BF16 = os.environ.get("MDE_GUIDE_BF16", "1") != "0"
 
 
-def _conv3x3_apply(x, weight, passes, want_stats, gx_slot=None):
+def _conv3x3_apply(x, weight, passes, want_stats, gx_slot=None, bn_slot=None):
     if weight.dtype != torch.float32:
         raise TypeError(f"conv3x3: the HIP kernels take a float32 weight, got {weight.dtype}")
     cin, cout = x.shape[1], weight.shape[0]
+    if bn_slot is not None:
+        return _Conv3x3.apply(x, weight, tuple(passes), want_stats, gx_slot, bn_slot)
     if (GUIDE_BF16 and cin == 3 and cout in (16, 32, 64) and passes[0] and x.dtype == torch.float32
             and _autocast_bf16(x) and not x.requires_grad
             and x.numel() < (1 << 31)):
@@ -997,14 +1034,14 @@
     return _Conv3x3.apply(x, weight, tuple(passes), want_stats, gx_slot)
 
 
-def conv3x3(x, weight, passes=(True, True, True), gx_slot=None):
+def conv3x3(x, weight, passes=(True, True, True), gx_slot=None, bn_slot=None):
     _gpu(x)
-    return _conv3x3_apply(x, weight, passes, False, gx_slot)[0]
-
-
-def conv3x3_stats(x, weight, passes=(True, True, True), gx_slot=None):
+    return _conv3x3_apply(x, weight, passes, False, gx_slot, bn_slot)[0]
+
+
+def conv3x3_stats(x, weight, passes=(True, True, True), gx_slot=None, bn_slot=None):
     _gpu(x)
-    y, stats = _conv3x3_apply(x, weight, passes, bool(passes[0]), gx_slot)
+    y, stats = _conv3x3_apply(x, weight, passes, bool(passes[0]), gx_slot, bn_slot)
     return y, (stats if stats.shape[1] > 0 else None)
 
 
@@ -1228,6 +1265,26 @@
             and c1.groups == 1 and c1.in_channels == c0.out_channels)
 
 
+BN_FOLD = int(os.environ.get("MDE_BN_FOLD", "1"))
+_BN_FOLD_SHAPES = {(16, 16): (True, 2), (3, 16): (False, 1), (3, 32): (False, 1)}
+
+
+def _bn_fold_slot(conv: nn.Conv2d, c1: nn.Conv2d, x, passes):
+    if not (BN_FOLD and passes is not None and torch.is_grad_enabled() and x.is_cuda
+            and x.dtype == torch.float32 and not _autocast_bf16(x)):
+        return None
+    key = (conv.in_channels, conv.out_channels)
+    dgrad, level = _BN_FOLD_SHAPES.get(key, (False, 1 << 30))
+    if (int(BN_FOLD) < level or passes[2] is not True or key[1] > _PW_BN_SUMS_MAX_CIN
+            or not (conv.weight.requires_grad or x.requires_grad)):
+        return None
+    if x.requires_grad and not (dgrad and passes[1] is True):
+        return None
+    if not pointwise_ok(c1, x):
+        return None
+    return BnFoldSlot()
+
+
 def run_sequential(seq: nn.Sequential, x):
     mods = list(seq)
     i = 0
@@ -1236,14 +1293,17 @@
         if x.is_cuda and _bnrelu_pw_at(mods, i, x.shape):
             want = mods[i + 1].training or not mods[i + 1].track_running_stats
             passes = conv3x3_passes(m, x)
+            slot = _bn_fold_slot(m, mods[i + 3], x, passes)
             if passes is not None and want:
-                y1, st1 = conv3x3_stats(x, m.weight, passes)
+                y1, st1 = conv3x3_stats(x, m.weight, passes, None, slot)
+            elif slot is not None:
+                y1, st1 = conv3x3(x, m.weight, passes, None, slot), None
             else:
                 y1, st1 = conv_nobias(m, x), None
             if pointwise_ok(mods[i + 3], y1):
                 b2 = mods[i + 4]
                 y2, st2 = bn_relu_pointwise(y1, mods[i + 1], m.bias, mods[i + 3], st1,
-                                            b2.training or not b2.track_running_stats)
+                                            b2.training or not b2.track_running_stats, slot)
                 x = batch_norm_act(y2, b2, b2.act, None, mods[i + 3].bias, st2)
                 i += 5
                 continue
@@ -1277,12 +1337,13 @@
     same = (m.stride == (1, 1) and m.dilation == (1, 1) and k[0] % 2 == 1 and k[1] % 2 == 1
             and m.padding == (k[0] // 2, k[1] // 2))
     passes = conv3x3_passes(m, x)
+    slot = _bn_fold_slot(m, c1, x, passes) if same else None
     if passes is not None:
-        y1, st1 = conv3x3_stats(x, m.weight, passes)
+        y1, st1 = conv3x3_stats(x, m.weight, passes, None, slot)
     else:
         y1, st1 = conv_nobias(m, x), None
     if same and pointwise_ok(c1, x):
-        y2, st2 = bn_relu_pointwise(y1, mods[1], m.bias, c1, st1, True)
+        y2, st2 = bn_relu_pointwise(y1, mods[1], m.bias, c1, st1, True, slot)
         return y2, st2, mods[4], c1.bias
     x1 = batch_norm_act(y1, mods[1], "relu", None, m.bias, st1)
     y2 = torch.nn.functional.conv2d(x1, c1.weight, None, c1.stride, c1.padding, c1.dilation,
```

Result: no change. 1010 images/s (median of 6 runs) (+0.7%).
